# bittremieux/ANN-SoLo

Measured on AMD Instinct MI355X. Metric: query spectra/sec + recall@k vs brute-force, open-mod search on MassIVE-KB, higher is better.
Workload: dtype f32; 1 GPU; configs[2]: MassIVE-KB-scale synthetic library (2100000 spectra, one charge-2 partition), ivfpq m=32 nlist=4096 nprobe=128 k=1024, open +-500 Da, shifted dot, fragment tol 0.02 Da; library_size=2100000, batch_per_gpu=32768, reference_default_batch_size=16384, global_batch=32768, index=ivfpq, nlist=4096, nprobe=128, k=1024, parallelism=single

## Files before the change

ann_solo_amd/csrc/coarse_sparse.hip:

```cpp
#include "common.hpp"
#include "ivf_kernels.hpp"

namespace asl {

constexpr int CS_TL = 32;
constexpr int CS_NW = 16;
constexpr int CS_CAP = 64;

__global__ __launch_bounds__(256) void list_nonzeros_kernel(const float *__restrict__ xq, int nq, int d,
                                                            int64_t ldq, uint2 *__restrict__ ent,
                                                            int32_t *__restrict__ cnt,
                                                            int *__restrict__ n_over) {
  const int q = blockIdx.x * 4 + (threadIdx.x >> 6), lane = threadIdx.x & 63;
  if (q >= nq) return;
  const float *row = xq + (size_t)q * ldq;
  uint2 *out = ent + (size_t)q * CS_CAP;
  int base = 0;
  for (int j0 = 0; j0 < d; j0 += 64) {
    const int j = j0 + lane;
    const float x = j < d ? row[j] : 0.0f;
    const unsigned long long m = __ballot(x != 0.0f);
    if (x != 0.0f) {
      const int t = base + __popcll(m & ((1ull << lane) - 1ull));
      if (t < CS_CAP) out[t] = make_uint2((uint32_t)j * (CS_TL * 4), __float_as_uint(x));
    }
    base += __popcll(m);
  }
  for (int t = base + lane; t < CS_CAP; t += 64) out[t] = make_uint2(0u, 0u);
  if (lane == 0) {
    cnt[q] = base <= CS_CAP ? base : -1 - base;
    if (base > CS_CAP) atomicAdd(n_over, 1);
  }
}

typedef float cs_f2 __attribute__((ext_vector_type(2)));
typedef __attribute__((address_space(3))) cs_f2 cs_lds_f2;

#define CS_NOP2 "s_nop 1\n\t"
#define CS_ADDR_(PRE, K, ED, I)                                                          \
  asm(PRE "v_add_u32_dpp %0, %1, %2 row_newbcast:" #K " row_mask:0xf bank_mask:0xf"     \
      : "=v"(ad[I])                                                                      \
      : "v"(ED), "v"(lane_off));
#define CS_ADDR(K, ED, I) CS_ADDR_("", K, ED, I)
#define CS_FMA(K, EV, I) CS_FMA_("", K, EV, I)
#define CS_FMA_(PRE, K, EV, I)                                                           \
  asm(PRE "v_fmac_f32_dpp %0, %1, %2 row_newbcast:" #K " row_mask:0xf bank_mask:0xf"    \
      : "+v"(acc0)                                                                   \
      : "v"(EV), "v"(cv[I].x));                                                      \
  asm("v_fmac_f32_dpp %0, %1, %2 row_newbcast:" #K " row_mask:0xf bank_mask:0xf"    \
      : "+v"(acc1)                                                                   \
      : "v"(EV), "v"(cv[I].y));
#define CS_BLOCK8(K0, K1, K2, K3, K4, K5, K6, K7, ED, EV)                                       \
  {                                                                                             \
    uint32_t ad[8];                                                                             \
    cs_f2 cv[8];                                                                                \
    CS_ADDR_(CS_NOP2, K0, ED, 0) CS_ADDR(K1, ED, 1) CS_ADDR(K2, ED, 2) CS_ADDR(K3, ED, 3)                 \
    CS_ADDR(K4, ED, 4) CS_ADDR(K5, ED, 5) CS_ADDR(K6, ED, 6) CS_ADDR(K7, ED, 7)                 \
    _Pragma("unroll") for (int i_ = 0; i_ < 8; ++i_) cv[i_] = *(const cs_lds_f2 *)(uintptr_t)ad[i_]; \
    CS_FMA_(CS_NOP2, K0, EV, 0) CS_FMA(K1, EV, 1) CS_FMA(K2, EV, 2) CS_FMA(K3, EV, 3)                     \
    CS_FMA(K4, EV, 4) CS_FMA(K5, EV, 5) CS_FMA(K6, EV, 6) CS_FMA(K7, EV, 7)                     \
  }
#define CS_BLOCK8A(ED, EV) CS_BLOCK8(0, 1, 2, 3, 4, 5, 6, 7, ED, EV)
#define CS_BLOCK8B(ED, EV) CS_BLOCK8(8, 9, 10, 11, 12, 13, 14, 15, ED, EV)

__global__ __launch_bounds__(64 * CS_NW) void coarse_sparse_kernel(
    const float *__restrict__ xq, int nq, int d, int64_t ldq, const uint2 *__restrict__ ent,
    const int32_t *__restrict__ cnt, const float *__restrict__ Ct, int nlist,
    float *__restrict__ scores, int ld, const int *__restrict__ n_over, int over_max) {
  if (*n_over > over_max) return;
  extern __shared__ __attribute__((aligned(16))) char cs_smem[];
  float *tile = reinterpret_cast<float *>(cs_smem);
  const int tid = threadIdx.x, lane = tid & 63, wave = tid >> 6;
  const int l0 = blockIdx.x * CS_TL;
  if (l0 + CS_TL <= nlist && (nlist & 3) == 0) {
    for (int i = tid; i < d * (CS_TL / 4); i += 64 * CS_NW) {
      const int dim = i >> 3, l4 = (i & 7) * 4;
      reinterpret_cast<float4 *>(tile)[i] =
          *reinterpret_cast<const float4 *>(Ct + (size_t)dim * nlist + l0 + l4);
    }
  } else {
    for (int i = tid; i < d * CS_TL; i += 64 * CS_NW) {
      const int dim = i >> 5, l = i & 31;
      tile[i] = l0 + l < nlist ? Ct[(size_t)dim * nlist + l0 + l] : 0.0f;
    }
  }
  __syncthreads();
  const int row = lane >> 4, j = lane & 15;
  const char *tile_lane = reinterpret_cast<const char *>(tile) + j * 8;
  const uint32_t lane_off =
      (uint32_t)(uintptr_t)(__attribute__((address_space(3))) char *)cs_smem + (uint32_t)(j * 8);
  const int groups = (nq + 3) >> 2;
  const int gper = (groups + gridDim.y - 1) / gridDim.y;
  const int g_lo = blockIdx.y * gper, g_hi = min(groups, g_lo + gper);
  uint32_t n_ed[4] = {0u, 0u, 0u, 0u}, n_ev[4] = {0u, 0u, 0u, 0u};
  int n_c = 0;
  auto fetch = [&](int g) {
    const int q = g * 4 + row;
    if (g < g_hi && q < nq) {
      n_c = cnt[q];
      const uint2 *e = ent + (size_t)q * CS_CAP + j;
#pragma unroll
      for (int u = 0; u < 4; ++u) {
        const uint2 x = e[16 * u];
        n_ed[u] = x.x;
        n_ev[u] = x.y;
      }
    } else {
      n_c = 0;
#pragma unroll
      for (int u = 0; u < 4; ++u) n_ed[u] = n_ev[u] = 0u;
    }
  };
  fetch(g_lo + wave);
  for (int g = g_lo + wave; g < g_hi; g += CS_NW) {
    const int q = g * 4 + row;
    const bool live = q < nq;
    const int c = n_c;
    const uint32_t ed[4] = {n_ed[0], n_ed[1], n_ed[2], n_ed[3]};
    const uint32_t ev[4] = {n_ev[0], n_ev[1], n_ev[2], n_ev[3]};
    fetch(g + CS_NW);
    float acc0 = 0.0f, acc1 = 0.0f;
    int cm = c < 0 ? 0 : c;
#pragma unroll
    for (int o = 32; o > 0; o >>= 1) cm = max(cm, __shfl_xor(cm, o, 64));
    cm = __builtin_amdgcn_readfirstlane(cm);
    if (cm > 0) { CS_BLOCK8A(ed[0], ev[0]) }
    if (cm > 8) { CS_BLOCK8B(ed[0], ev[0]) }
    if (cm > 16) { CS_BLOCK8A(ed[1], ev[1]) }
    if (cm > 24) { CS_BLOCK8B(ed[1], ev[1]) }
    if (cm > 32) { CS_BLOCK8A(ed[2], ev[2]) }
    if (cm > 40) { CS_BLOCK8B(ed[2], ev[2]) }
    if (cm > 48) { CS_BLOCK8A(ed[3], ev[3]) }
    if (cm > 56) { CS_BLOCK8B(ed[3], ev[3]) }
    if (__ballot(c < 0)) {
      if (c < 0) {
        acc0 = acc1 = 0.0f;
        const float *xr = xq + (size_t)q * ldq;
        for (int k = 0; k < d; ++k) {
          const float vv = xr[k];
          if (vv != 0.0f) {
            const float2 cc = *reinterpret_cast<const float2 *>(tile_lane + (size_t)k * (CS_TL * 4));
            acc0 = __builtin_fmaf(vv, cc.x, acc0);
            acc1 = __builtin_fmaf(vv, cc.y, acc1);
          }
        }
      }
    }
    if (live) {
      const int l = l0 + 2 * j;
      float *o = scores + (size_t)q * ld + l;
      if (l + 1 < nlist && (ld & 1) == 0) {
        *reinterpret_cast<float2 *>(o) = make_float2(acc0, acc1);
      } else {
        if (l < nlist) o[0] = acc0;
        if (l + 1 < nlist) o[1] = acc1;
      }
    }
  }
}

int list_nonzeros(const float *xq, int nq, int d, int64_t ldq, uint2 *ent, int32_t *cnt, int *n_over) {
  if (nq <= 0) return ASL_OK;
  hipLaunchKernelGGL(list_nonzeros_kernel, dim3((unsigned)cdiv(nq, 4)), dim3(256), 0, stream(), xq,
                     nq, d, ldq > 0 ? ldq : (int64_t)d, ent, cnt, n_over);
  ASL_CHECK_LAUNCH();
  return ASL_OK;
}

bool coarse_sparse_supported(int d, int nlist) {
  return d >= 1 && (size_t)d * CS_TL * 4 <= 150 * 1024 && nlist >= 1;
}

__global__ void transpose_f32_kernel(const float *__restrict__ in, int rows, int cols,
                                     float *__restrict__ out) {
  __shared__ float t[32][33];
  const int bx = blockIdx.x * 32, by = blockIdx.y * 32;
  const int x = threadIdx.x & 31, y0 = threadIdx.x >> 5;
  for (int y = y0; y < 32; y += 8)
    if (by + y < rows && bx + x < cols) t[y][x] = in[(size_t)(by + y) * cols + bx + x];
  __syncthreads();
  for (int y = y0; y < 32; y += 8)
    if (bx + y < cols && by + x < rows) out[(size_t)(bx + y) * rows + by + x] = t[x][y];
}

int transpose_f32(const float *in, int rows, int cols, float *out) {
  if (rows <= 0 || cols <= 0) return ASL_OK;
  hipLaunchKernelGGL(transpose_f32_kernel, dim3((unsigned)cdiv(cols, 32), (unsigned)cdiv(rows, 32)),
                     dim3(256), 0, stream(), in, rows, cols, out);
  ASL_CHECK_LAUNCH();
  return ASL_OK;
}

int coarse_sparse(const float *xq, int nq, int d, const float *Ct, int nlist, uint2 *ent,
                  int32_t *cnt, int *n_over, int over_max, float *scores, int ld, int64_t ldq) {
  if (ldq <= 0) ldq = d;
  if (nq <= 0) return ASL_OK;
  HIP_TRY(hipMemsetAsync(n_over, 0, sizeof(int), stream()));
  hipLaunchKernelGGL(list_nonzeros_kernel, dim3((unsigned)cdiv(nq, 4)), dim3(256), 0, stream(), xq,
                     nq, d, ldq, ent, cnt, n_over);
  ASL_CHECK_LAUNCH();
  const int tiles = (int)cdiv(nlist, CS_TL);
  int parts = std::max(1, std::min((512 + tiles - 1) / tiles, (nq + 4 * CS_NW - 1) / (4 * CS_NW)));
  const size_t lds = (size_t)d * CS_TL * 4;
  HIP_TRY(hipFuncSetAttribute((const void *)coarse_sparse_kernel,
                              hipFuncAttributeMaxDynamicSharedMemorySize, (int)lds));
  hipLaunchKernelGGL(coarse_sparse_kernel, dim3(tiles, parts), dim3(64 * CS_NW), lds, stream(), xq, nq, d,
                     ldq, ent, cnt, Ct, nlist, scores, ld, n_over, over_max);
  ASL_CHECK_LAUNCH();
  return ASL_OK;
}

int coarse_sparse_cap() { return CS_CAP; }

}
```

ann_solo_amd/csrc/encode.hip:

```cpp
#include "common.hpp"

namespace asl {

__device__ __forceinline__ uint32_t rotl32(uint32_t x, int r) {
  return (x << r) | (x >> (32 - r));
}

__device__ __forceinline__ uint32_t murmur3_round(uint32_t h1, uint32_t k1) {
  k1 *= 0xcc9e2d51u;
  k1 = rotl32(k1, 15);
  k1 *= 0x1b873593u;
  h1 ^= k1;
  h1 = rotl32(h1, 13);
  return h1 * 5 + 0xe6546b64u;
}

__device__ __forceinline__ uint32_t murmur3_decimal_small(int v, uint32_t seed) {
  const bool neg = v < 0;
  uint32_t u = neg ? (uint32_t)(-(long long)v) : (uint32_t)v;
  int nd = 1;
  nd += u >= 10u;
  nd += u >= 100u;
  nd += u >= 1000u;
  nd += u >= 10000u;
  nd += u >= 100000u;
  nd += u >= 1000000u;
  nd += u >= 10000000u;
  nd += u >= 100000000u;
  const int len = nd + (neg ? 1 : 0);
  uint32_t w0 = neg ? (uint32_t)'-' : 0u, w1 = 0u, w2 = 0u;
#pragma unroll
  for (int j = 0; j < 9; ++j) {
    if (j < nd) {
      const uint32_t qd = u / 10u;
      const uint32_t ch = (uint32_t)'0' + (u - qd * 10u);
      u = qd;
      const int pos = len - 1 - j;
      const uint32_t sh = ch << ((pos & 3) * 8);
      w0 |= (pos >> 2) == 0 ? sh : 0u;
      w1 |= (pos >> 2) == 1 ? sh : 0u;
      w2 |= (pos >> 2) == 2 ? sh : 0u;
    }
  }
  uint32_t h1 = seed;
  if (len >= 4) h1 = murmur3_round(h1, w0);
  if (len >= 8) h1 = murmur3_round(h1, w1);
  const uint32_t tail = len >= 8 ? w2 : (len >= 4 ? w1 : w0);
  if (len & 3) {
    uint32_t k1 = tail & (0xFFFFFFFFu >> (32 - 8 * (len & 3)));
    k1 *= 0xcc9e2d51u;
    k1 = rotl32(k1, 15);
    k1 *= 0x1b873593u;
    h1 ^= k1;
  }
  h1 ^= (uint32_t)len;
  h1 ^= h1 >> 16;
  h1 *= 0x85ebca6bu;
  h1 ^= h1 >> 13;
  h1 *= 0xc2b2ae35u;
  h1 ^= h1 >> 16;
  return h1;
}

__device__ uint32_t murmur3_decimal(long long v, uint32_t seed) {
  if (v > -1000000000ll && v < 1000000000ll) return murmur3_decimal_small((int)v, seed);
  unsigned char buf[24];
  int len = 0;
  unsigned long long u = v < 0 ? (unsigned long long)(-(v + 1)) + 1ull : (unsigned long long)v;
  unsigned char tmp[24];
  int nd = 0;
  do {
    tmp[nd++] = (unsigned char)('0' + (u % 10));
    u /= 10;
  } while (u);
  if (v < 0) buf[len++] = '-';
  for (int i = nd - 1; i >= 0; --i) buf[len++] = tmp[i];
  const uint32_t c1 = 0xcc9e2d51u, c2 = 0x1b873593u;
  uint32_t h1 = seed;
  int nblocks = len >> 2;
  for (int i = 0; i < nblocks; ++i) {
    uint32_t k1 = (uint32_t)buf[4 * i] | ((uint32_t)buf[4 * i + 1] << 8) |
                  ((uint32_t)buf[4 * i + 2] << 16) | ((uint32_t)buf[4 * i + 3] << 24);
    k1 *= c1;
    k1 = rotl32(k1, 15);
    k1 *= c2;
    h1 ^= k1;
    h1 = rotl32(h1, 13);
    h1 = h1 * 5 + 0xe6546b64u;
  }
  uint32_t k1 = 0;
  int t = nblocks * 4;
  int rem = len & 3;
  if (rem == 3) k1 ^= (uint32_t)buf[t + 2] << 16;
  if (rem >= 2) k1 ^= (uint32_t)buf[t + 1] << 8;
  if (rem >= 1) {
    k1 ^= buf[t];
    k1 *= c1;
    k1 = rotl32(k1, 15);
    k1 *= c2;
    h1 ^= k1;
  }
  h1 ^= (uint32_t)len;
  h1 ^= h1 >> 16;
  h1 *= 0x85ebca6bu;
  h1 ^= h1 >> 13;
  h1 *= 0xc2b2ae35u;
  h1 ^= h1 >> 16;
  return h1;
}

__device__ long long np_floor_div_bin(double a, double b) {
  const double q0 = a / b;
  if (b > 0.0 && fabs(q0) < 2147483648.0) {
    double q = floor(q0);
    if (fma(-q, b, a) < 0.0) q -= 1.0;
    return (long long)q;
  }
  double mod = fmod(a, b);
  double div = (a - mod) / b;
  if (mod != 0.0 && ((b < 0) != (mod < 0))) div -= 1.0;
  double fd;
  if (div != 0.0) {
    fd = floor(div);
    if (div - fd > 0.5) fd += 1.0;
  } else {
    fd = copysign(0.0, a / b);
  }
  return (long long)floor(fd);
}

constexpr int ENC_WAVES = 4;
constexpr int QE_CAP = 64;
constexpr int QE_DIM_SHIFT = 7;

template <bool ENTRIES>
__global__ __launch_bounds__(64 * ENC_WAVES) void encode_kernel(
    const float *__restrict__ mz, const float *__restrict__ inten,
    const int32_t *__restrict__ offsets, int32_t n, double min_bound, double bin_size,
    int32_t hash_len, uint32_t seed, int norm, float *__restrict__ out, uint2 *__restrict__ ent,
    int32_t *__restrict__ ent_cnt, int *__restrict__ n_over) {
  extern __shared__ __attribute__((aligned(16))) char smem[];
  const int wave = threadIdx.x >> 6, lane = threadIdx.x & 63;
  const int spec = blockIdx.x * ENC_WAVES + wave;
  float *vec = reinterpret_cast<float *>(smem) + (size_t)wave * hash_len;
  if (spec >= n) return;

  for (int i = lane; i < hash_len; i += 64) vec[i] = 0.0f;
  const int p0 = offsets[spec], p1 = offsets[spec + 1];
  for (int base = p0; base < p1; base += 64) {
    const int p = base + lane;
    const int cnt = min(64, p1 - base);
    const bool live = lane < cnt;
    int idx = -1 - lane;
    float val = 0.0f;
    if (live) {
      long long b = np_floor_div_bin((double)mz[p] - min_bound, bin_size);
      idx = (int)(murmur3_decimal(b, seed) % (uint32_t)hash_len);
      val = inten[p];
    }
    int rank = 0;
    for (int j = 0; j < cnt; ++j) {
      const int o = __builtin_amdgcn_readlane(idx, j);
      rank += (o == idx && j < lane) ? 1 : 0;
    }
    for (int r = 0; __ballot(live && rank >= r) != 0ull; ++r) {
      if (live && rank == r) vec[idx] += val;
      __builtin_amdgcn_wave_barrier();
    }
  }
  float nrm = 1.0f;
  if (norm) {
    float acc = 0.0f;
    for (int i0 = 0; i0 < hash_len; i0 += 64) {
      const int i = i0 + lane;
      const float v = i < hash_len ? vec[i] : 0.0f;
      unsigned long long m = __ballot(v != 0.0f);
      while (m) {
        const int l = __builtin_ctzll(m);
        m &= m - 1ull;
        const float x = __builtin_bit_cast(
            float, __builtin_amdgcn_readlane(__builtin_bit_cast(int, v), l));
        acc = __builtin_fmaf(x, x, acc);
      }
    }
    nrm = __builtin_sqrtf(acc);
  }
  if (!ENTRIES) {
    float *row = out + (size_t)spec * hash_len;
    for (int i = lane; i < hash_len; i += 64) row[i] = norm ? vec[i] / nrm : vec[i];
    return;
  }
  uint2 *row = ent + (size_t)spec * QE_CAP;
  int have = 0;
  for (int i0 = 0; i0 < hash_len; i0 += 64) {
    const int i = i0 + lane;
    float x = i < hash_len ? vec[i] : 0.0f;
    if (norm) x = x / nrm;
    if (!(i < hash_len)) x = 0.0f;
    const unsigned long long m = __ballot(x != 0.0f);
    if (x != 0.0f) {
      const int t = have + __popcll(m & ((1ull << lane) - 1ull));
      if (t < QE_CAP) row[t] = make_uint2((uint32_t)i << QE_DIM_SHIFT, __float_as_uint(x));
    }
    have += __popcll(m);
  }
  for (int t = have + lane; t < QE_CAP; t += 64) row[t] = make_uint2(0u, 0u);
  if (lane == 0) {
    ent_cnt[spec] = have <= QE_CAP ? have : -1 - have;
    if (have > QE_CAP && n_over) atomicAdd(n_over, 1);
  }
}

template <bool ENTRIES>
static int encode_launch(const float *mz, const float *inten, const int32_t *offsets, int32_t n,
                         double min_bound, double bin_size, int32_t hash_len, uint32_t seed, int norm,
                         float *out, uint2 *ent, int32_t *ent_cnt, int *n_over) {
  size_t lds = (size_t)ENC_WAVES * hash_len * sizeof(float);
  if (lds > 160 * 1024) return fail(ASL_ERR_CAPACITY, "encode: hash_len %d too large for LDS", hash_len);
  dim3 grid((unsigned)cdiv(n, ENC_WAVES));
  if (lds > 64 * 1024)
    HIP_TRY(hipFuncSetAttribute((const void *)encode_kernel<ENTRIES>,
                                hipFuncAttributeMaxDynamicSharedMemorySize, (int)lds));
  hipLaunchKernelGGL(encode_kernel<ENTRIES>, grid, dim3(64 * ENC_WAVES), lds, stream(), mz, inten,
                     offsets, n, min_bound, bin_size, hash_len, seed, norm, out, ent, ent_cnt, n_over);
  ASL_CHECK_LAUNCH();
  return ASL_OK;
}

int encode_device(const float *mz, const float *inten, const int32_t *offsets, int32_t n,
                  double min_bound, double bin_size, int32_t hash_len, uint32_t seed,
                  int norm, float *out) {
  if (n == 0) return ASL_OK;
  ProfScope ps("encode");
  return encode_launch<false>(mz, inten, offsets, n, min_bound, bin_size, hash_len, seed, norm, out,
                              nullptr, nullptr, nullptr);
}

int encode_entries_device(const float *mz, const float *inten, const int32_t *offsets, int32_t n,
                          double min_bound, double bin_size, int32_t hash_len, uint32_t seed, int norm,
                          uint2 *ent, int32_t *cnt, int *n_over) {
  if (n == 0) return ASL_OK;
  ProfScope ps("encode");
  return encode_launch<true>(mz, inten, offsets, n, min_bound, bin_size, hash_len, seed, norm, nullptr,
                             ent, cnt, n_over);
}

}

using namespace asl;

static uint32_t host_rotl32(uint32_t x, int r) { return (x << r) | (x >> (32 - r)); }
static uint32_t host_murmur3(const unsigned char *key, int len, uint32_t seed) {
  const uint32_t c1 = 0xcc9e2d51u, c2 = 0x1b873593u;
  uint32_t h1 = seed;
  int nblocks = len / 4;
  for (int i = 0; i < nblocks; i++) {
    uint32_t k1;
    memcpy(&k1, key + 4 * i, 4);
    k1 *= c1;
    k1 = host_rotl32(k1, 15);
    k1 *= c2;
    h1 ^= k1;
    h1 = host_rotl32(h1, 13);
    h1 = h1 * 5 + 0xe6546b64u;
  }
  const unsigned char *tail = key + nblocks * 4;
  uint32_t k1 = 0;
  switch (len & 3) {
    case 3: k1 ^= (uint32_t)tail[2] << 16; [[fallthrough]];
    case 2: k1 ^= (uint32_t)tail[1] << 8; [[fallthrough]];
    case 1:
      k1 ^= tail[0];
      k1 *= c1;
      k1 = host_rotl32(k1, 15);
      k1 *= c2;
      h1 ^= k1;
  }
  h1 ^= (uint32_t)len;
  h1 ^= h1 >> 16;
  h1 *= 0x85ebca6bu;
  h1 ^= h1 >> 13;
  h1 *= 0xc2b2ae35u;
  h1 ^= h1 >> 16;
  return h1;
}

extern "C" {

int32_t asl_hash_idx(int64_t bin_idx, int32_t hash_len, uint32_t seed) {
  if (hash_len <= 0) return -1;
  char buf[32];
  int len = snprintf(buf, sizeof buf, "%lld", (long long)bin_idx);
  return (int32_t)(host_murmur3((const unsigned char *)buf, len, seed) % (uint32_t)hash_len);
}

int asl_get_dim(double min_mz, double max_mz, double bin_size, int64_t *n_bins,
                double *start_dim, double *end_dim) {
  if (!(bin_size > 0)) return fail(ASL_ERR_INVALID, "get_dim: bin_size must be > 0");
  auto pymod = [](double a, double b) {
    double m = fmod(a, b);
    if (m != 0.0 && ((b < 0) != (m < 0))) m += b;
    return m;
  };
  double s = min_mz - pymod(min_mz, bin_size);
  double e = max_mz + bin_size - pymod(max_mz, bin_size);
  if (start_dim) *start_dim = s;
  if (end_dim) *end_dim = e;
  if (n_bins) *n_bins = (int64_t)nearbyint((e - s) / bin_size);
  return ASL_OK;
}

int asl_encode_batch(const float *mz, const float *intensity, const int32_t *offsets,
                     int32_t n, double min_bound, double bin_size, int32_t hash_len,
                     uint32_t seed, int norm, float *out) {
  clear_error();
  if (n < 0 || hash_len <= 0 || !(bin_size > 0))
    return fail(ASL_ERR_INVALID, "encode_batch: bad n/hash_len/bin_size");
  if (n == 0) return ASL_OK;
  if (!offsets || !out) return fail(ASL_ERR_INVALID, "encode_batch: null offsets/out");
  ASL_TRY(ensure_device());
  int32_t last = 0;
  if (is_device_ptr(offsets)) {
    HIP_TRY(hipMemcpyAsync(&last, offsets + n, sizeof(int32_t), hipMemcpyDeviceToHost, stream()));
    ASL_TRY(sync_stream());
  } else {
    last = offsets[n];
  }
  if (last > 0 && (!mz || !intensity)) return fail(ASL_ERR_INVALID, "encode_batch: null peaks");
  In<float> dmz, din;
  In<int32_t> doff;
  Out<float> dout;
  ASL_TRY(dmz.init(mz, (size_t)last));
  ASL_TRY(din.init(intensity, (size_t)last));
  ASL_TRY(doff.init(offsets, (size_t)n + 1));
  ASL_TRY(dout.init(out, (size_t)n * hash_len));
  ASL_TRY(encode_device(dmz.d, din.d, doff.d, n, min_bound, bin_size, hash_len, seed, norm,
                        dout.d));
  ASL_TRY(dout.finish());
  if (dout.to_host() || dmz.own.p || din.own.p || doff.own.p) ASL_TRY(sync_stream());
  return ASL_OK;
}

int asl_encode_entries_batch(const float *mz, const float *intensity, const int32_t *offsets,
                             int32_t n, int32_t n_peaks, double min_bound, double bin_size,
                             int32_t hash_len, uint32_t seed, int norm, uint32_t *entries,
                             int32_t *counts, int32_t *n_over) {
  clear_error();
  if (n < 0 || hash_len <= 0 || !(bin_size > 0))
    return fail(ASL_ERR_INVALID, "encode_entries_batch: bad n/hash_len/bin_size");
  if (n == 0) return ASL_OK;
  if (!offsets || !entries || !counts) return fail(ASL_ERR_INVALID, "encode_entries_batch: null offsets/entries/counts");
  ASL_TRY(ensure_device());
  if (!is_device_ptr(entries) || !is_device_ptr(counts) || (n_over && !is_device_ptr(n_over)))
    return fail(ASL_ERR_INVALID, "encode_entries_batch: entries / counts / n_over must be device memory");
  int32_t last = n_peaks;
  if (last < 0) {
    if (is_device_ptr(offsets)) {
      HIP_TRY(hipMemcpyAsync(&last, offsets + n, sizeof(int32_t), hipMemcpyDeviceToHost, stream()));
      ASL_TRY(sync_stream());
    } else {
      last = offsets[n];
    }
  }
  if (last > 0 && (!mz || !intensity)) return fail(ASL_ERR_INVALID, "encode_entries_batch: null peaks");
  In<float> dmz, din;
  In<int32_t> doff;
  ASL_TRY(dmz.init(mz, (size_t)last));
  ASL_TRY(din.init(intensity, (size_t)last));
  ASL_TRY(doff.init(offsets, (size_t)n + 1));
  ASL_TRY(encode_entries_device(dmz.d, din.d, doff.d, n, min_bound, bin_size, hash_len, seed, norm,
                                reinterpret_cast<uint2 *>(entries), counts, n_over));
  if (dmz.own.p || din.own.p || doff.own.p) ASL_TRY(sync_stream());
  return ASL_OK;
}

}
```

ann_solo_amd/csrc/index.hpp:

```cpp
#pragma once
#include "common.hpp"
#include "flat_postings.hpp"
#include "ivf_kernels.hpp"

namespace asl {

constexpr size_t SCORE_CHUNK_BYTES = (size_t)1 << 30;
constexpr int FLAT_KEYS_SLACK = 768;

struct ShardScratch {
  DevBuf<float> x_all, cD, cD_all, Dp, Dr, Dtmp, Dfin, x3, cD3;
  DevBuf<int32_t> cI, cI_all, cI3, mine, everyone;
  DevBuf<int64_t> Ip, Ir, Im;
  DevBuf<uint2> e_loc, e_all, e3;
  DevBuf<int32_t> c_loc, c_all, c3, over;
  DevBuf<int64_t> Kp, Hs, Hr, Ko, Bs, Br, Xs, Xr, Mn, rowlist, K3;
  DevBuf<int32_t> need, flag, Fl, rmap;
  DevBuf<unsigned int> cursor;
};

enum IndexRows { ROWS_ORDERED = 0, ROWS_SET, ROWS_SET_RAW, ROWS_KEYS };

struct IndexSearch {
  int nq = 0;
  const float *xq = nullptr;
  int k = 0, nprobe = 0;
  float *D = nullptr;
  int64_t *I64 = nullptr;
  int32_t *I32 = nullptr;
  const float *pre_D = nullptr;
  const int32_t *pre_I = nullptr;
  const uint2 *pre_ent = nullptr;
  const int32_t *pre_cnt = nullptr;
  const int *gate = nullptr;
  int rows = ROWS_ORDERED;
  const IndexPostFilter *post = nullptr;
  uint64_t serial = 0, gen = 0;
  const IndexWindow *win = nullptr;
  const uint8_t *sel_keep = nullptr;
  int64_t sel_n = 0;
  bool rows_filtered = false;
};

}

struct asl_index {
  int d = 0, nlist = 0, kind = 0, pq_m = 0, pq_bits = 8, ksub = 0, dsub = 0;
  int niter = 25;
  bool trained = false;
  bool by_residual = true;
  int64_t ntotal = 0;
  int64_t n_store = 0;
  int shard_rank = 0, shard_world = 1;
  asl::DevBuf<float> centroids, codebooks;
  asl::DevBuf<float> codebooks_t;
  bool cbt_ready = false;
  asl::DevBuf<float> centroids_t;
  bool cent_t_ready = false;
  asl::DevBuf<float> kmeans_ct;
  asl::DevBuf<uint2> scan_ent;
  asl::DevBuf<int32_t> scan_cnt;
  asl::DevBuf<int> scan_over;
  asl::DevBuf<uint2> cs_ent;
  asl::DevBuf<int32_t> cs_cnt;
  asl::DevBuf<int> cs_over;
  asl::DevBuf<float> vecs;
  asl::DevBuf<int32_t> vlist;
  asl::DevBuf<int32_t> vids;
  bool has_vids = false;
  asl::DevBuf<uint8_t> codes_add;
  asl::DevBuf<uint8_t> codes;
  asl::DevBuf<int32_t> ids, list_offsets;
  std::vector<int32_t> h_list_offsets;
  asl::DevBuf<uint8_t> codes_tiled;
  asl::DevBuf<int32_t> ids_tiled, tile_offsets;
  asl::DevBuf<int2> idpay;
  int64_t n_tile_slots = 0;
  uint64_t pay_serial = 0;
  uint64_t pay_gen = 0;
  int64_t pay_n = 0;
  bool idpay_ready = false;
  bool has_tiles = false;
  asl::DevBuf<uint8_t> wcodes_tiled;
  asl::DevBuf<int32_t> wids_tiled;
  asl::DevBuf<float> wkey_tiled;
  bool win_ready = false;
  uint64_t win_serial = 0;
  uint64_t win_gen = 0;
  int window_scan = 0;
  asl::DevBuf<int2> win_ranges;
  asl::DevBuf<float> wf_key;
  asl::DevBuf<uint8_t> codes_mm;
  uint32_t mm_plane = 0;
  bool mm_ready = false;
  bool scan_mmajor = true;
  asl::DevBuf<unsigned long long> sel_words, wsel_words;
  bool sel_ready = false, wsel_ready = false;
  uint64_t sel_serial = 0, sel_gen = 0, wsel_serial = 0, wsel_gen = 0;
  asl::DevBuf<uint8_t> selector;
  bool has_selector = false;
  uint64_t selector_gen = 0;
  int64_t n_blocks = 0;
  asl::DevBuf<int32_t> blk_offsets;
  asl::DevBuf<uint32_t> blk_base;
  asl::DevBuf<uint32_t> inv_tab;
  asl::DevBuf<char> inv_data;
  bool has_inv = false;
  int flat_storage = ASL_FLAT_F32;
  int inv_layout = 0;
  int nnz_max = 0;
  int tab_stride = 0;
  asl::DevBuf<uint8_t> inv_tab8;
  asl::DevBuf<uint16_t> inv_cnt16;
  int scan_variant = 0;
  int unordered = 0;
  bool lists_dirty = true;
  int agreed_k = -1, agreed_np = -1, agreed_world = -1, agreed_val = -1;
  int refine_k = 0;
  bool refine_rows = false;
  bool refine_bad = false;
  int64_t r_n = 0;
  asl::DevBuf<uint16_t> r_dim;
  asl::DevBuf<float> r_val;
  asl::DevBuf<uint8_t> r_cnt;
  asl::DevBuf<int32_t> ws_short;
  asl::DevBuf<float> ws_scores, coarse_D, ws_x;
  asl::DevBuf<int32_t> coarse_I, ws_assign;
  asl::DevBuf<float> zero_D;
  asl::DevBuf<uint32_t> bitmap;
  asl::DevBuf<uint64_t> ws_upper;
  asl::ShardScratch shard;
};

namespace asl {

int index_shape_check(const char *who, int d, int nlist, int kind, int pq_m, int pq_bits);
constexpr int PQ_TILED_MAX_D = 1020;
inline bool ivf_kind(int kind) { return kind == ASL_INDEX_IVFFLAT || kind == ASL_INDEX_IVFPQ; }
inline bool window_mode(const asl_index *ix) { return ix->window_scan || ix->kind == ASL_INDEX_WINFLAT; }
inline bool tiled_index(const asl_index *ix) {
  return ix->kind == ASL_INDEX_IVFPQ && ix->pq_m == 32 && ix->ksub == 256 && ix->d <= PQ_TILED_MAX_D;
}
inline FlatPostings postings_view(const asl_index *ix) {
  FlatPostings P;
  P.layout = ix->has_inv ? ix->inv_layout : 0, P.d = ix->d, P.nlist = ix->nlist, P.n_blocks = ix->n_blocks;
  P.list_offsets = ix->list_offsets.p, P.blk_offsets = ix->blk_offsets.p, P.blk_base = ix->blk_base.p;
  if (P.layout == 2) P.tab8 = ix->inv_tab8.p, P.cnt16 = ix->inv_cnt16.p;
  else P.tab32 = ix->inv_tab.p;
  P.tab_stride = ix->tab_stride, P.seg_bytes = ix->inv_data.p, P.ids = ix->ids.p;
  return P;
}
int assign_ip(asl_index *ix, const float *x, int64_t ld, int64_t n, const float *cent, int k, int d,
              int32_t *assign_dev);
int build_lists(asl_index *ix);
int build_postings(asl_index *ix, const int32_t *order_dev, int64_t n, const std::vector<int32_t> &blk_off,
                   const std::vector<int32_t> &pos_blk, const std::vector<uint16_t> &pos_loc);
int winflat_layout(asl_index *ix, bool keyed, const float *key, uint64_t serial, uint64_t gen);
const char *window_unsupported(const asl_index *ix);
int window_install(asl_index *ix, int64_t n, const float *key, uint64_t serial, uint64_t gen = 0);
int post_filter_pairs(asl_index *ix, const IndexPostFilter &p, uint64_t serial, uint64_t gen,
                      const int32_t *slot_ids, int64_t nslots);
int selector_words(asl_index *ix, const IndexSearch &rq, bool window, const unsigned long long **words);
int index_search_device(asl_index *ix, IndexSearch &rq);
int index_nprobe(const asl_index *ix, int nprobe);
int index_prepare(asl_index *ix);
int coarse_search(asl_index *ix, const float *xq, int nq, int nprobe, float *out_D, int32_t *out_I, uint2 *ent_out,
                  int32_t *cnt_out, bool *have_ent);
int index_window_prepare(asl_index *ix, uint64_t serial, uint64_t gen, const float *key, int64_t n, int nq,
                         int nprobe);
int index_refine_k(const asl_index *ix);
int coarse_scores_all(asl_index *ix, const float *xq, int m, float *scores, uint2 *ent = nullptr, int32_t *cnt = nullptr);
int index_codebooks_transposed(asl_index *ix);
int index_codes_mmajor(asl_index *ix);
int index_zero_coarse(asl_index *ix, size_t n, const float **zeros);

}
```

ann_solo_amd/csrc/index_search.hip:

```cpp
#include <algorithm>

#include "index.hpp"

namespace asl {

static int coarse_transposed(asl_index *ix) {
  if (ix->cent_t_ready) return ASL_OK;
  ASL_TRY(ix->centroids_t.reserve((size_t)ix->nlist * ix->d));
  ASL_TRY(transpose_f32(ix->centroids.p, ix->nlist, ix->d, ix->centroids_t.p));
  ix->cent_t_ready = true;
  return ASL_OK;
}

int coarse_scores_all(asl_index *ix, const float *xq, int m, float *scores, uint2 *ent, int32_t *cnt) {
  const int nlist = ix->nlist, d = ix->d;
  const bool sparse = ix->scan_variant == 0 && coarse_sparse_supported(d, nlist);
  const int over_max = m / 64;
  if (sparse) {
    ASL_TRY(coarse_transposed(ix));
    ASL_TRY(ix->cs_ent.reserve((size_t)m * coarse_sparse_cap()));
    ASL_TRY(ix->cs_cnt.reserve((size_t)m));
    ASL_TRY(ix->cs_over.reserve(1));
    ASL_TRY(coarse_sparse(xq, m, d, ix->centroids_t.p, nlist, ent ? ent : ix->cs_ent.p, cnt ? cnt : ix->cs_cnt.p,
                          ix->cs_over.p, over_max, scores, nlist));
  }
  return gemm_nt_f32(xq, ix->centroids.p, scores, m, nlist, d, d, d, nlist, sparse ? ix->cs_over.p : nullptr, over_max);
}

int coarse_search(asl_index *ix, const float *xq, int nq, int nprobe, float *out_D, int32_t *out_I, uint2 *ent_out,
                  int32_t *cnt_out, bool *have_ent) {
  const int nlist = ix->nlist, d = ix->d;
  if (have_ent) *have_ent = false;
  if (!out_D) {
    ASL_TRY(ix->coarse_D.reserve((size_t)nq * nprobe));
    ASL_TRY(ix->coarse_I.reserve((size_t)nq * nprobe));
    out_D = ix->coarse_D.p;
    out_I = ix->coarse_I.p;
  }
  int rows = (int)std::min<int64_t>(nq, std::max<int64_t>(1, (int64_t)(SCORE_CHUNK_BYTES / ((size_t)nlist * 4))));
  ASL_TRY(ix->ws_scores.reserve((size_t)rows * nlist));
  const bool sparse = ix->scan_variant == 0 && coarse_sparse_supported(d, nlist);
  for (int r0 = 0; r0 < nq; r0 += rows) {
    const int m = std::min(rows, nq - r0);
    {
      ProfScope ps("coarse_gemm");
      ASL_TRY(coarse_scores_all(ix, xq + (size_t)r0 * d, m, ix->ws_scores.p, ent_out ? ent_out + (size_t)r0 * 64 : nullptr,
                                cnt_out ? cnt_out + (size_t)r0 : nullptr));
    }
    {
      ProfScope ps("coarse_select");
      ASL_TRY(row_topk(ix->ws_scores.p, nlist, m, nlist, nprobe, nullptr, 0, nullptr, nullptr, 0,
                       out_D + (size_t)r0 * nprobe, nullptr, out_I + (size_t)r0 * nprobe, nprobe));
    }
  }
  if (have_ent) *have_ent = sparse && coarse_sparse_cap() == 64 && ((ent_out && cnt_out) || nq <= rows);
  return ASL_OK;
}

static bool postings_ok(const asl_index *ix, int k, int nprobe) {
  return ix->has_inv && ix->scan_variant == 0 && flat_inv_supported(ix->d, k, nprobe);
}
static bool tiled_shape_ok(const asl_index *ix, int k, int nprobe) {
  return ix->scan_variant == 0 && tiled_index(ix) && pq_scan_tiled_supported(ix->pq_m, ix->ksub, k, nprobe);
}
static bool keys_fit(int k) { return k + FLAT_KEYS_SLACK <= TK_MAX_K; }

static int clamp_nprobe(const asl_index *ix, int *nprobe, const char *who) {
  *nprobe = std::max(1, std::min(*nprobe, ix->nlist));
  if (*nprobe > TK_MAX_K) return fail(ASL_ERR_CAPACITY, "%s: nprobe=%d > %d", who, *nprobe, TK_MAX_K);
  return ASL_OK;
}

static int count_scanned(const asl_index *ix, const int32_t *cI, int nq, int nprobe) {
  if (!prof_counts()) return ASL_OK;
  if (unsigned long long *acc = prof_scanned_dev())
    ASL_TRY(scanned_count(cI, (int64_t)nq * nprobe, ix->list_offsets.p, acc));
  return ASL_OK;
}

struct SearchPlan {
  int unordered = 0;
  int nprobe = 0;
  bool refine = false;
  int k_scan = 0;
  bool use_inv = false, tiled = false;
};

static int validate_winflat(asl_index *ix, const IndexSearch &rq, const SearchPlan &pl) {
  if (rq.gate || rq.pre_I || rq.pre_D)
    return fail(ASL_ERR_STATE, "a window-exact index has no probe lists: no preassigned or gated search");
  if (rq.pre_ent && !rq.xq) return fail(ASL_ERR_STATE, "a window-exact index takes no entry-list-only queries");
  if (pl.unordered == 2) return fail(ASL_ERR_STATE, "packed-key rows are not served by a window-exact index");
  if (rq.sel_keep && !rq.win)
    return fail(ASL_ERR_STATE, "a window-exact index takes a selection through its key column (NaN: unselected), "
                               "not a selector");
  if (rq.win && !rq.win->q_pmz) return fail(ASL_ERR_INVALID, "window scan: null precursor m/z");
  if (rq.nq <= 0) return ASL_OK;
  if (!rq.xq) return fail(ASL_ERR_INVALID, "search: null queries");
  if (rq.k <= 0) return fail(ASL_ERR_CAPACITY, "search: k=%d outside 1..%d", rq.k, TK_MAX_K - FLAT_KEYS_SLACK);
  if (!keys_fit(rq.k))
    return fail(ASL_ERR_STATE, "a window-exact index holds k <= %d (k=%d)", TK_MAX_K - FLAT_KEYS_SLACK, rq.k);
  if (!flat_inv_supported(ix->d, rq.k, 1))
    return fail(ASL_ERR_STATE, "a window-exact index is searched by the postings scan, which holds d <= 4096 (d=%d)", ix->d);
  ASL_TRY(build_lists(ix));
  if (ix->n_store > 0 && !ix->has_inv && ix->d <= 65535 && ix->nnz_max == 0)
    return fail(ASL_ERR_STATE, "a window-exact index of all-zero vectors has no postings to scan");
  if (ix->n_store > 0 && !ix->has_inv)
    return fail(ASL_ERR_STATE, "a window-exact index needs sparse vectors: its postings are built when the most "
                               "non-zeros of a vector (%d), times 8, stay below d=%d", ix->nnz_max, ix->d);
  if (rq.win && !ix->win_ready)
    return fail(ASL_ERR_STATE, "window scan: no window key (asl_index_set_window_key), or vectors were added "
                               "since it was set");
  return ASL_OK;
}

static int validate(asl_index *ix, const IndexSearch &rq, SearchPlan &pl) {
  const int k = rq.k;
  pl.unordered = rq.rows == ROWS_KEYS ? 2 : rq.rows == ROWS_SET_RAW ? 1 : ix->unordered;
  if (ix->kind == ASL_INDEX_WINFLAT) return validate_winflat(ix, rq, pl);
  pl.refine = ix->kind == ASL_INDEX_IVFPQ && ix->refine_k > k && ix->refine_rows && pl.unordered == 0;
  if (rq.win) {
    if (const char *why = window_unsupported(ix)) return fail(ASL_ERR_STATE, "%s", why);
    if (ix->scan_variant != 0)
      return fail(ASL_ERR_STATE, "the window scan needs the layout-specific scan (scan_variant 0), not the generic kernels");
    if (!keys_fit(k)) return fail(ASL_ERR_STATE, "the window scan holds k <= %d (k=%d)", TK_MAX_K - FLAT_KEYS_SLACK, k);
    if (rq.gate || pl.unordered == 2 || pl.refine)
      return fail(ASL_ERR_STATE, "the window scan takes no gate, packed keys or exact re-rank");
    if (!rq.win->q_pmz) return fail(ASL_ERR_INVALID, "window scan: null precursor m/z");
  }
  if (rq.sel_keep) {
    if (ix->kind == ASL_INDEX_FLAT) return fail(ASL_ERR_STATE, "a selector needs an IVF index (not a Flat index)");
    if (ix->shard_world > 1 || ix->has_vids) return fail(ASL_ERR_STATE, "a selector does not run on a sharded index");
    if (ix->scan_variant != 0)
      return fail(ASL_ERR_STATE, "a selector needs the layout-specific scan (scan_variant 0), not the generic kernels");
    if (!keys_fit(k)) return fail(ASL_ERR_STATE, "a selected search holds k <= %d (k=%d)", TK_MAX_K - FLAT_KEYS_SLACK, k);
    if (rq.gate || pl.unordered == 2 || (rq.pre_ent && !rq.xq))
      return fail(ASL_ERR_STATE, "a selected search takes no gate, packed keys or entry-list-only queries");
    if (pl.refine) return fail(ASL_ERR_STATE, "a selected search does not run with the exact re-rank");
    if (rq.sel_n != ix->ntotal)
      return fail(ASL_ERR_INVALID, "selector: %lld flags for %lld vectors", (long long)rq.sel_n, (long long)ix->ntotal);
  }
  if (rq.nq <= 0) return ASL_OK;
  if (rq.pre_ent && (!rq.pre_cnt || !rq.pre_I || (!rq.xq && !rq.pre_D) || ix->kind == ASL_INDEX_FLAT))
    return fail(ASL_ERR_STATE, "entry-list search: needs the counts, the caller's probe lists (with their scores when "
                               "no dense rows are given) and an IVF index");
  if (!rq.xq && !rq.pre_ent) return fail(ASL_ERR_INVALID, "search: null queries");
  if (rq.gate && (!rq.pre_I || ix->kind == ASL_INDEX_FLAT))
    return fail(ASL_ERR_STATE, "gated search: needs the caller's probe lists and an IVF index");
  if (!ix->trained) return fail(ASL_ERR_STATE, "search: index is not trained");
  if (k <= 0 || k > TK_MAX_K_PASSES) return fail(ASL_ERR_CAPACITY, "search: k=%d outside 1..%d", k, TK_MAX_K_PASSES);
  const bool ents_only = rq.pre_ent && !rq.xq;
  pl.nprobe = rq.nprobe;
  pl.k_scan = k;
  if (k > TK_MAX_K && (rq.gate || ents_only || pl.unordered == 2))
    return fail(ASL_ERR_STATE, "search: k=%d > %d is served from dense queries only (no packed keys, "
                               "entry-list-only queries or gates)", k, TK_MAX_K);
  if (ix->kind == ASL_INDEX_FLAT) {
    if (pl.unordered == 2) return fail(ASL_ERR_STATE, "packed-key rows need an IVF index");
    return ASL_OK;
  }
  ASL_TRY(clamp_nprobe(ix, &pl.nprobe, "search"));
  ASL_TRY(build_lists(ix));
  if (k > TK_MAX_K) return ASL_OK;
  if (ix->kind == ASL_INDEX_IVFFLAT) {
    pl.use_inv = postings_ok(ix, k, pl.nprobe);
    if (pl.unordered == 2 && !(pl.use_inv && rq.I64 && keys_fit(k)))
      return fail(ASL_ERR_STATE, "packed-key rows need the postings scan of IVF-Flat (sparse vectors, k <= 1280) and an int64 output");
    if (rq.gate && !pl.use_inv) return fail(ASL_ERR_STATE, "gated search: needs the postings scan of IVF-Flat");
    if (ents_only && !pl.use_inv) return fail(ASL_ERR_STATE, "entry-list search: needs the postings scan of IVF-Flat");
    if (rq.sel_keep && !pl.use_inv)
      return fail(ASL_ERR_STATE, "a selector needs the postings scan of IVF-Flat (sparse vectors, nprobe <= 1024), "
                                 "not dense rows");
    return ASL_OK;
  }
  if (rq.gate && pl.refine) return fail(ASL_ERR_STATE, "gated search: not with the exact re-rank");
  if (ents_only && pl.refine) return fail(ASL_ERR_STATE, "entry-list search: not with the exact re-rank (it reads the dense queries)");
  if (pl.refine) {
    if (ix->refine_bad)
      return fail(ASL_ERR_CAPACITY, "search: refine is unavailable, a stored vector has more than %d non-zeros",
                  refine_stride());
    if (ix->r_n != ix->ntotal)
      return fail(ASL_ERR_STATE, "search: refine rows cover %lld of %lld vectors (enable refine before add)",
                  (long long)ix->r_n, (long long)ix->ntotal);
    pl.k_scan = std::min(ix->refine_k, (int)TK_MAX_K);
  }
  pl.tiled = ix->has_tiles && tiled_shape_ok(ix, pl.k_scan, pl.nprobe);
  if (pl.unordered == 2 && !(pl.tiled && rq.I64))
    return fail(ASL_ERR_STATE, "packed-key rows need the tiled IVF-PQ scan (m = 32, 8 bits) and an int64 output");
  if (rq.gate && !pl.tiled) return fail(ASL_ERR_STATE, "gated search: needs the tiled IVF-PQ scan");
  if (ents_only && !pl.tiled) return fail(ASL_ERR_STATE, "entry-list search: needs the tiled IVF-PQ scan (m = 32, 8 bits)");
  if (rq.sel_keep && !pl.tiled)
    return fail(ASL_ERR_STATE, "a selector needs the tiled IVF-PQ scan (m = 32, 8 bits, nprobe <= 1024)");
  if (rq.win && !pl.tiled) return fail(ASL_ERR_STATE, "the window scan needs the tiled IVF-PQ scan (m = 32, 8 bits)");
  if (rq.win && !ix->win_ready)
    return fail(ASL_ERR_STATE, "window scan: no window key (asl_index_set_window_key), or the lists changed "
                               "since it was set");
  return ASL_OK;
}

static int query_entries(asl_index *ix, const IndexSearch &rq, bool own_ent, const uint2 **q_ent,
                         const int32_t **q_cnt) {
  *q_ent = rq.pre_ent;
  *q_cnt = rq.pre_cnt;
  if (!rq.pre_ent && own_ent) {
    *q_ent = ix->cs_ent.p;
    *q_cnt = ix->cs_cnt.p;
  } else if (!rq.pre_ent) {
    ASL_TRY(ix->scan_ent.reserve((size_t)rq.nq * 64));
    ASL_TRY(ix->scan_cnt.reserve((size_t)rq.nq));
    ASL_TRY(ix->scan_over.reserve(1));
    ASL_TRY(list_nonzeros(rq.xq, rq.nq, ix->d, ix->d, ix->scan_ent.p, ix->scan_cnt.p, ix->scan_over.p));
    *q_ent = ix->scan_ent.p;
    *q_cnt = ix->scan_cnt.p;
  }
  return ASL_OK;
}

static int take_post_filter(asl_index *ix, IndexSearch &rq, int mode, const int32_t *slot_ids, int64_t nslots,
                            ScanPostFilter &pf) {
  pf = ScanPostFilter();
  if (!rq.post) return ASL_OK;
  const IndexPostFilter &p = *rq.post;
  if (!(mode == 1 && rq.I32 && !rq.I64 && !rq.D && !rq.gate && keys_fit(rq.k)) || !p.payload || !p.q_pmz || !p.count ||
      p.n != ix->ntotal || ix->has_vids) return ASL_OK;
  ASL_TRY(post_filter_pairs(ix, p, rq.serial, rq.gen, slot_ids, nslots));
  pf = {.idpay = ix->idpay.p, .q_pmz = p.q_pmz, .count = p.count, .tol = p.tol, .mode = p.mode, .charge = p.charge};
  rq.rows_filtered = true;
  return ASL_OK;
}

static int pass_bounds(asl_index *ix, const IndexSearch &rq, uint64_t **upper) {
  *upper = nullptr;
  if (rq.k <= TK_MAX_K) return ASL_OK;
  ASL_TRY(ix->ws_upper.reserve((size_t)rq.nq));
  *upper = ix->ws_upper.p;
  return ASL_OK;
}

static int search_gemm_topk(asl_index *ix, const IndexSearch &rq, const int32_t *cI, int nprobe) {
  const int nq = rq.nq, k = rq.k, d = ix->d;
  const int64_t n = ix->n_store;
  const bool ivf = cI != nullptr;
  uint64_t *upper;
  ASL_TRY(pass_bounds(ix, rq, &upper));
  int words = 0;
  if (ivf) {
    words = (ix->nlist + 31) / 32;
    ASL_TRY(ix->bitmap.reserve((size_t)nq * words));
    ASL_TRY(probe_bitmap(cI, nq, nprobe, ix->bitmap.p, words));
    if (n > 0) ASL_TRY(count_scanned(ix, cI, nq, nprobe));
  }
  const int64_t ncol = std::max<int64_t>(n, 1);
  int rows = (int)std::min<int64_t>(nq, std::max<int64_t>(1, (int64_t)(SCORE_CHUNK_BYTES / ((size_t)ncol * 4))));
  ASL_TRY(ix->ws_scores.reserve((size_t)rows * ncol));
  auto out_at = [&](auto *base, int64_t r0, int c0) { return base ? base + (size_t)r0 * k + c0 : nullptr; };
  for (int r0 = 0; r0 < nq; r0 += rows) {
    const int m = std::min(rows, nq - r0);
    ProfScope ps("scan");
    if (n > 0)
      ASL_TRY(gemm_nt_f32(rq.xq + (size_t)r0 * d, ix->vecs.p, ix->ws_scores.p, m, (int)n, d, d, d, (int)n));
    for (int c0 = 0; c0 < k; c0 += TK_MAX_K) {
      const int kp = std::min<int>(TK_MAX_K, k - c0);
      ASL_TRY(row_topk(ix->ws_scores.p, n, m, (int)n, kp, ix->has_vids ? ix->vids.p : nullptr, 0,
                       ivf ? ix->vlist.p : nullptr, ivf ? ix->bitmap.p + (size_t)r0 * words : nullptr, words,
                       out_at(rq.D, r0, c0), out_at(rq.I64, r0, c0), out_at(rq.I32, r0, c0), k,
                       c0 ? upper + r0 : nullptr, upper ? upper + r0 : nullptr));
    }
  }
  return upper ? sync_stream() : ASL_OK;
}

static int search_ivfflat(asl_index *ix, IndexSearch &rq, const SearchPlan &pl) {
  const int nq = rq.nq, nprobe = pl.nprobe;
  bool own_ent = false;
  if (!rq.pre_I) ASL_TRY(coarse_search(ix, rq.xq, nq, nprobe, nullptr, nullptr, nullptr, nullptr, &own_ent));
  const int32_t *cI = rq.pre_I ? rq.pre_I : ix->coarse_I.p;
  if (!pl.use_inv) return search_gemm_topk(ix, rq, cI, nprobe);
  const uint2 *q_ent;
  const int32_t *q_cnt;
  ASL_TRY(query_entries(ix, rq, own_ent, &q_ent, &q_cnt));
  const int mode_ = pl.unordered ? pl.unordered : (rq.rows != ROWS_ORDERED ? 1 : 0);
  ScanPostFilter pf;
  ASL_TRY(take_post_filter(ix, rq, mode_, ix->ids.p, ix->n_store, pf));
  const unsigned long long *sel = nullptr;
  if (rq.sel_keep) ASL_TRY(selector_words(ix, rq, false, &sel));
  {
    ProfScope ps("scan");
    FlatScan fs;
    fs.xq = rq.xq, fs.ent = q_ent, fs.ent_cnt = q_cnt, fs.nq = nq, fs.k = rq.k;
    fs.coarse_I = cI, fs.nprobe = nprobe, fs.gate = rq.gate, fs.post = pf, fs.sel = sel;
    fs.D = rq.D, fs.I64 = rq.I64, fs.I32 = rq.I32, fs.set_mode = mode_;
    ASL_TRY(flat_inv_scan(postings_view(ix), fs));
  }
  return rq.gate ? ASL_OK : count_scanned(ix, cI, nq, nprobe);
}

static int search_winflat(asl_index *ix, IndexSearch &rq, const SearchPlan &pl) {
  const int nq = rq.nq;
  const uint2 *q_ent;
  const int32_t *q_cnt;
  ASL_TRY(query_entries(ix, rq, false, &q_ent, &q_cnt));
  const int mode_ = (pl.unordered || rq.rows != ROWS_ORDERED) ? 1 : 0;
  ASL_TRY(ix->win_ranges.reserve((size_t)nq));
  {
    ProfScope ps("window_ranges");
    const IndexWindow *w = rq.win;
    ASL_TRY(winflat_runs(w ? w->q_pmz : nullptr, nq, ix->wf_key.p, ix->n_store, w ? w->charge : 0, w ? w->tol : 0.0,
                         w ? w->mode : ASL_TOL_DA, ix->win_ranges.p,
                         prof_counts() ? prof_scanned_dev() : nullptr));
  }
  FlatScan fs;
  fs.xq = rq.xq, fs.ent = q_ent, fs.ent_cnt = q_cnt, fs.nq = nq, fs.k = rq.k;
  fs.D = rq.D, fs.I64 = rq.I64, fs.I32 = rq.I32, fs.set_mode = mode_;
  fs.ranges.range = ix->win_ranges.p;
  fs.ranges.row_len = (rq.win && mode_ == 1) ? rq.win->row_len : nullptr;
  rq.rows_filtered = fs.ranges.row_len != nullptr;
  ProfScope ps("scan");
  return flat_inv_scan(postings_view(ix), fs);
}

int index_codebooks_transposed(asl_index *ix) {
  if (ix->cbt_ready) return ASL_OK;
  const size_t ncb = (size_t)ix->pq_m * ix->ksub * ix->dsub;
  std::vector<float> h((size_t)ncb), ht((size_t)ncb);
  ASL_TRY(ix->codebooks.download(h.data(), ncb));
  ASL_TRY(sync_stream());
  for (int m = 0; m < ix->pq_m; m++)
    for (int c = 0; c < ix->ksub; c++)
      for (int t = 0; t < ix->dsub; t++)
        ht[((size_t)m * ix->dsub + t) * ix->ksub + c] = h[((size_t)m * ix->ksub + c) * ix->dsub + t];
  ASL_TRY(ix->codebooks_t.upload(ht.data(), ncb));
  ASL_TRY(sync_stream());
  ix->cbt_ready = true;
  return ASL_OK;
}

int index_zero_coarse(asl_index *ix, size_t n, const float **zeros) {
  if (n > ix->zero_D.cap) {
    ASL_TRY(ix->zero_D.reserve(n));
    HIP_TRY(hipMemsetAsync(ix->zero_D.p, 0, n * sizeof(float), stream()));
  }
  *zeros = ix->zero_D.p;
  return ASL_OK;
}

int index_codes_mmajor(asl_index *ix) {
  if (ix->mm_ready) return ASL_OK;
  const int64_t ntiles = ix->n_tile_slots / 64;
  const uint64_t plane = ((((uint64_t)ntiles * 64 + 127) / 128) | 1u) * 128;
  if (plane * (uint64_t)ix->pq_m >= (1ull << 32)) return ASL_OK;
  ASL_TRY(ix->codes_mm.reserve((size_t)plane * (size_t)ix->pq_m));
  ASL_TRY(mmajor_codes(ix->codes_tiled.p, ntiles, (uint32_t)plane, ix->codes_mm.p));
  ASL_TRY(sync_stream());
  ix->mm_plane = (uint32_t)plane;
  ix->mm_ready = true;
  return ASL_OK;
}

static int scan_pq_tiled(asl_index *ix, IndexSearch &rq, const SearchPlan &pl, const float *cD, const int32_t *cI,
                         bool own_ent) {
  const int nq = rq.nq, nprobe = pl.nprobe;
  ASL_TRY(index_codebooks_transposed(ix));
  const uint2 *q_ent;
  const int32_t *q_cnt;
  ASL_TRY(query_entries(ix, rq, own_ent, &q_ent, &q_cnt));
  const int mode_ = pl.unordered ? pl.unordered : (rq.rows != ROWS_ORDERED ? 1 : 0);
  ScanPostFilter pf;
  ScanRanges rg;
  if (rq.win) {
    const IndexWindow &wq = *rq.win;
    ASL_TRY(ix->win_ranges.reserve((size_t)nq * nprobe));
    ProfScope ps("window_ranges");
    ASL_TRY(window_ranges(wq.q_pmz, nq, cI, nprobe, ix->list_offsets.p, ix->tile_offsets.p, ix->wkey_tiled.p,
                          wq.charge, wq.tol, wq.mode, ix->win_ranges.p,
                          prof_counts() ? prof_scanned_dev() : nullptr));
    rg.range = ix->win_ranges.p;
    rg.row_len = mode_ == 1 ? wq.row_len : nullptr;
    rq.rows_filtered = rg.row_len != nullptr;
  } else {
    ASL_TRY(take_post_filter(ix, rq, mode_, ix->ids_tiled.p, ix->n_tile_slots, pf));
  }
  const unsigned long long *sel = nullptr;
  if (rq.sel_keep) ASL_TRY(selector_words(ix, rq, rq.win != nullptr, &sel));
  const bool mm = ix->scan_mmajor && !rq.win && !rq.sel_keep && !rq.gate && ix->shard_world == 1 && !ix->has_vids;
  if (mm) ASL_TRY(index_codes_mmajor(ix));
  const bool use_mm = mm && ix->mm_ready;
  ProfScope ps("scan");
  return pq_scan_v3(rq.xq, nq, ix->d, ix->codebooks_t.p, ix->dsub, cD, cI,
                    nprobe, ix->list_offsets.p, ix->tile_offsets.p,
                    rq.win ? ix->wcodes_tiled.p : ix->codes_tiled.p, rq.win ? ix->wids_tiled.p : ix->ids_tiled.p,
                    rq.k, rq.D, rq.I64, rq.I32, mode_, q_ent, q_cnt, rq.gate, &pf, &rg, sel,
                    use_mm ? ix->codes_mm.p : nullptr, use_mm ? ix->mm_plane : 0u);
}

static int search_ivfpq(asl_index *ix, IndexSearch &rq, const SearchPlan &pl) {
  const int nq = rq.nq, nprobe = pl.nprobe;
  bool own_ent = false;
  if (!rq.pre_D) ASL_TRY(coarse_search(ix, rq.xq, nq, nprobe, nullptr, nullptr, nullptr, nullptr, &own_ent));
  const float *cD = rq.pre_D ? rq.pre_D : ix->coarse_D.p;
  const int32_t *cI = rq.pre_D ? rq.pre_I : ix->coarse_I.p;
  if (!ix->by_residual) ASL_TRY(index_zero_coarse(ix, (size_t)nq * nprobe, &cD));
  uint64_t *upper = nullptr;
  if (pl.tiled) {
    ASL_TRY(scan_pq_tiled(ix, rq, pl, cD, cI, own_ent));
  } else {
    const int k = rq.k;
    ASL_TRY(pass_bounds(ix, rq, &upper));
    auto out_at = [&](auto *base, int c0) { return base ? base + c0 : nullptr; };
    ProfScope ps("scan");
    for (int c0 = 0; c0 < k; c0 += TK_MAX_K) {
      const int kp = std::min<int>(TK_MAX_K, k - c0);
      ASL_TRY(pq_scan(rq.xq, nq, ix->d, ix->codebooks.p, ix->pq_m, ix->ksub, ix->dsub, cD, cI, nprobe,
                      ix->list_offsets.p, ix->ids.p, ix->codes.p, kp, out_at(rq.D, c0), out_at(rq.I64, c0),
                      out_at(rq.I32, c0), k, c0 ? upper : nullptr, upper));
    }
  }
  if (!rq.gate && !rq.win) ASL_TRY(count_scanned(ix, cI, nq, nprobe));
  return upper ? sync_stream() : ASL_OK;
}

static int search_ivfpq_refined(asl_index *ix, IndexSearch &rq, const SearchPlan &pl) {
  IndexSearch scan = rq;
  scan.k = pl.k_scan;
  ASL_TRY(ix->ws_short.reserve((size_t)rq.nq * scan.k));
  scan.D = nullptr;
  scan.I64 = nullptr;
  scan.I32 = ix->ws_short.p;
  scan.rows = ROWS_SET;
  scan.post = nullptr;
  ASL_TRY(search_ivfpq(ix, scan, pl));
  ProfScope ps("refine");
  return refine_topk(rq.xq, rq.nq, ix->d, ix->ws_short.p, nullptr, scan.k, ix->r_dim.p, ix->r_val.p, ix->r_cnt.p,
                     ix->r_n, rq.k, rq.D, rq.I64, rq.I32);
}

int index_search_device(asl_index *ix, IndexSearch &rq) {
  rq.rows_filtered = false;
  SearchPlan pl;
  ASL_TRY(validate(ix, rq, pl));
  if (rq.nq <= 0) return ASL_OK;
  if (ix->kind == ASL_INDEX_FLAT) return search_gemm_topk(ix, rq, nullptr, 0);
  if (ix->kind == ASL_INDEX_WINFLAT) return search_winflat(ix, rq, pl);
  if (ix->kind == ASL_INDEX_IVFFLAT) return search_ivfflat(ix, rq, pl);
  return pl.refine ? search_ivfpq_refined(ix, rq, pl) : search_ivfpq(ix, rq, pl);
}

int index_window_prepare(asl_index *ix, uint64_t serial, uint64_t gen, const float *key, int64_t n, int nq,
                         int nprobe) {
  if (!ix->trained) return fail(ASL_ERR_STATE, "search: index is not trained");
  if (ix->kind != ASL_INDEX_WINFLAT) ASL_TRY(build_lists(ix));
  if (ix->lists_dirty || !ix->win_ready || ix->win_serial != serial || ix->win_gen != gen) {
    ASL_TRY(pipeline_drain());
    ASL_TRY(window_install(ix, n, key, serial, gen));
  }
  return ix->win_ranges.reserve((size_t)std::max(nq, 1) * std::max(1, std::min(nprobe, ix->nlist)));
}

int index_nprobe(const asl_index *ix, int nprobe) {
  return !ivf_kind(ix->kind) ? 0 : std::max(1, std::min(nprobe, ix->nlist));
}
int index_prepare(asl_index *ix) {
  if (!ix->trained) return fail(ASL_ERR_STATE, "search: index is not trained");
  if (!ivf_kind(ix->kind)) return ASL_OK;
  if (coarse_sparse_supported(ix->d, ix->nlist)) ASL_TRY(coarse_transposed(ix));
  return build_lists(ix);
}
int index_refine_k(const asl_index *ix) {
  return (ix->refine_rows && !ix->refine_bad && ix->r_n == ix->ntotal) ? ix->refine_k : 0;
}

template <class F>
static int with_staged_rows(float *D, int64_t *I, size_t n, bool staged_in, F call) {
  Out<float> dD;
  Out<int64_t> dI;
  ASL_TRY(dD.init(D, n));
  ASL_TRY(dI.init(I, n));
  ASL_TRY(call(dD.d, dI.d));
  ASL_TRY(dD.finish());
  ASL_TRY(dI.finish());
  if (dD.to_host() || dI.to_host() || staged_in) ASL_TRY(sync_stream());
  return ASL_OK;
}

}

using namespace asl;

extern "C" {

int asl_index_supports_keys(asl_index_t *ix, int32_t k, int32_t nprobe) {
  if (!ix) return 0;
  nprobe = std::max(1, std::min(nprobe, ix->nlist));
  if (ix->kind == ASL_INDEX_IVFFLAT) {
    if (ix->lists_dirty && ix->trained && (ensure_device() != ASL_OK || build_lists(ix) != ASL_OK)) return 0;
    return postings_ok(ix, k, nprobe) && keys_fit(k);
  }
  if (ix->kind != ASL_INDEX_IVFPQ) return 0;
  return tiled_shape_ok(ix, k, nprobe) && keys_fit(k);
}

int asl_index_coarse(asl_index_t *ix, int32_t nq, const float *xq, int32_t nprobe,
                     float *coarse_D, int32_t *coarse_I) {
  clear_error();
  if (!ix || !ivf_kind(ix->kind) || !ix->trained)
    return fail(ASL_ERR_STATE, "coarse: trained IVF index required");
  if (nq <= 0) return ASL_OK;
  ASL_TRY(clamp_nprobe(ix, &nprobe, "coarse"));
  In<float> dq;
  ASL_TRY(dq.init(xq, (size_t)nq * ix->d));
  ASL_TRY(coarse_search(ix, dq.d, nq, nprobe, nullptr, nullptr, nullptr, nullptr, nullptr));
  if (coarse_D)
    HIP_TRY(hipMemcpyAsync(coarse_D, ix->coarse_D.p, (size_t)nq * nprobe * 4, hipMemcpyDefault, stream()));
  if (coarse_I)
    HIP_TRY(hipMemcpyAsync(coarse_I, ix->coarse_I.p, (size_t)nq * nprobe * 4, hipMemcpyDefault, stream()));
  return sync_stream();
}

int asl_index_postings_work(asl_index_t *ix, int32_t nq, const float *xq, int32_t nprobe,
                            int64_t *bytes, int64_t *lines) {
  clear_error();
  if (!ix || ix->kind != ASL_INDEX_IVFFLAT || !ix->trained)
    return fail(ASL_ERR_STATE, "postings_work: trained IVF-Flat index required");
  if (bytes) *bytes = 0;
  if (lines) *lines = 0;
  if (nq <= 0) return ASL_OK;
  ASL_TRY(ensure_device());
  ASL_TRY(clamp_nprobe(ix, &nprobe, "postings_work"));
  ASL_TRY(build_lists(ix));
  if (!ix->has_inv) return fail(ASL_ERR_STATE, "postings_work: the index holds no postings (dense vectors)");
  In<float> dq;
  ASL_TRY(dq.init(xq, (size_t)nq * ix->d));
  ASL_TRY(coarse_search(ix, dq.d, nq, nprobe, nullptr, nullptr, nullptr, nullptr, nullptr));
  DevBuf<unsigned long long> acc;
  ASL_TRY(acc.reserve(2));
  HIP_TRY(hipMemsetAsync(acc.p, 0, 16, stream()));
  ASL_TRY(flat_postings_work(postings_view(ix), dq.d, nq, ix->coarse_I.p, nprobe, acc.p));
  unsigned long long h[2] = {0, 0};
  ASL_TRY(acc.download(h, 2));
  ASL_TRY(sync_stream());
  if (bytes) *bytes = (int64_t)h[0];
  if (lines) *lines = (int64_t)h[1];
  return ASL_OK;
}

int asl_index_pq_lut(asl_index_t *ix, int32_t nq, const float *xq, float *lut) {
  clear_error();
  if (!ix || ix->kind != ASL_INDEX_IVFPQ || !ix->trained)
    return fail(ASL_ERR_STATE, "pq_lut: trained IVF-PQ index required");
  if (nq <= 0) return ASL_OK;
  In<float> dq;
  Out<float> dl;
  ASL_TRY(dq.init(xq, (size_t)nq * ix->d));
  ASL_TRY(dl.init(lut, (size_t)nq * ix->pq_m * ix->ksub));
  ASL_TRY(pq_lut(dq.d, nq, ix->d, ix->codebooks.p, ix->pq_m, ix->ksub, ix->dsub, dl.d));
  ASL_TRY(dl.finish());
  return sync_stream();
}

int asl_index_search(asl_index_t *ix, int32_t nq, const float *xq, int32_t k, int32_t nprobe,
                     float *D, int64_t *I) {
  clear_error();
  if (!ix) return fail(ASL_ERR_INVALID, "search: null index");
  if (nq <= 0) return ASL_OK;
  if (!xq || !I) return fail(ASL_ERR_INVALID, "search: null xq / I");
  ASL_TRY(ensure_device());
  In<float> dq;
  ASL_TRY(dq.init(xq, (size_t)nq * ix->d));
  return with_staged_rows(D, I, (size_t)nq * k, dq.own.p, [&](float *dD, int64_t *dI) {
    IndexSearch rq{.nq = nq, .xq = dq.d, .k = k, .nprobe = nprobe, .D = dD, .I64 = dI};
    return index_search_device(ix, rq);
  });
}

int asl_index_search_window(asl_index_t *ix, int32_t nq, const float *xq, const double *q_pmz, int32_t charge,
                            double tol, int32_t mode, int32_t k, int32_t nprobe, float *D, int64_t *I) {
  clear_error();
  ASL_TRY(ensure_device());
  if (!ix) return fail(ASL_ERR_INVALID, "search_window: null index");
  if (nq <= 0) return ASL_OK;
  if (!xq || !q_pmz || !I) return fail(ASL_ERR_INVALID, "search_window: null xq / q_pmz / I");
  if (mode != ASL_TOL_DA && mode != ASL_TOL_PPM && mode != ASL_TOL_INTERVAL)
    return fail(ASL_ERR_INVALID, "search_window: mode must be Da, ppm or interval");
  if (ix->kind != ASL_INDEX_WINFLAT)
    if (const char *why = window_unsupported(ix)) return fail(ASL_ERR_STATE, "%s", why);
  if (!ix->trained) return fail(ASL_ERR_STATE, "search: index is not trained");
  if (ix->kind != ASL_INDEX_WINFLAT || !ix->lists_dirty) ASL_TRY(build_lists(ix));
  if (!ix->win_ready || (ix->kind == ASL_INDEX_WINFLAT && ix->lists_dirty))
    return fail(ASL_ERR_STATE, "search_window: no window key (asl_index_set_window_key), or the lists changed since");
  In<float> dq;
  In<double> dp;
  ASL_TRY(dq.init(xq, (size_t)nq * ix->d));
  ASL_TRY(dp.init(q_pmz, (size_t)nq * (mode == ASL_TOL_INTERVAL ? 2 : 1)));
  return with_staged_rows(D, I, (size_t)nq * k, dq.own.p || dp.own.p, [&](float *dD, int64_t *dI) {
    IndexWindow w{.q_pmz = dp.d, .tol = tol, .mode = mode, .charge = charge};
    IndexSearch rq{.nq = nq, .xq = dq.d, .k = k, .nprobe = nprobe, .D = dD, .I64 = dI, .win = &w};
    return index_search_device(ix, rq);
  });
}

int asl_index_set_selector(asl_index_t *ix, int64_t n, const uint8_t *keep) {
  clear_error();
  ASL_TRY(ensure_device());
  if (!ix) return fail(ASL_ERR_INVALID, "set_selector: null index");
  if (n == 0 || !keep) {
    ix->has_selector = false;
    return ASL_OK;
  }
  if (n != ix->ntotal)
    return fail(ASL_ERR_INVALID, "set_selector: %lld flags for %lld vectors", (long long)n, (long long)ix->ntotal);
  if (ivf_kind(ix->kind) && ix->trained) ASL_TRY(build_lists(ix));
  ix->has_selector = false;
  ASL_TRY(ix->selector.reserve((size_t)n));
  HIP_TRY(hipMemcpyAsync(ix->selector.p, keep, (size_t)n, hipMemcpyDefault, stream()));
  ASL_TRY(sync_stream());
  ix->has_selector = true;
  ++ix->selector_gen;
  return ASL_OK;
}

int asl_index_search_selected(asl_index_t *ix, int32_t nq, const float *xq, const double *q_pmz, int32_t charge,
                              double tol, int32_t mode, int32_t k, int32_t nprobe, float *D, int64_t *I) {
  clear_error();
  ASL_TRY(ensure_device());
  if (!ix) return fail(ASL_ERR_INVALID, "search_selected: null index");
  if (nq <= 0) return ASL_OK;
  if (!xq || !I) return fail(ASL_ERR_INVALID, "search_selected: null xq / I");
  if (q_pmz && mode != ASL_TOL_DA && mode != ASL_TOL_PPM && mode != ASL_TOL_INTERVAL)
    return fail(ASL_ERR_INVALID, "search_selected: mode must be Da, ppm or interval");
  if (ix->kind == ASL_INDEX_FLAT) return fail(ASL_ERR_STATE, "a selector needs an IVF index (not a Flat index)");
  if (ix->kind == ASL_INDEX_WINFLAT)
    return fail(ASL_ERR_STATE, "search_selected: a window-exact index takes a selection through its key column "
                               "(NaN: unselected), not a selector");
  if (!ix->trained) return fail(ASL_ERR_STATE, "search: index is not trained");
  ASL_TRY(build_lists(ix));
  if (!ix->has_selector)
    return fail(ASL_ERR_STATE, "search_selected: no selector (asl_index_set_selector), or the lists changed since "
                               "it was set");
  if (q_pmz) {
    if (const char *why = window_unsupported(ix)) return fail(ASL_ERR_STATE, "%s", why);
    if (!ix->win_ready)
      return fail(ASL_ERR_STATE, "search_selected: no window key (asl_index_set_window_key), or the lists changed since");
  }
  In<float> dq;
  In<double> dp;
  ASL_TRY(dq.init(xq, (size_t)nq * ix->d));
  if (q_pmz) ASL_TRY(dp.init(q_pmz, (size_t)nq * (mode == ASL_TOL_INTERVAL ? 2 : 1)));
  return with_staged_rows(D, I, (size_t)nq * k, dq.own.p || dp.own.p, [&](float *dD, int64_t *dI) {
    IndexWindow w{.q_pmz = dp.d, .tol = tol, .mode = mode, .charge = charge};
    IndexSearch rq{.nq = nq, .xq = dq.d, .k = k, .nprobe = nprobe, .D = dD, .I64 = dI, .serial = 0,
                   .gen = ix->selector_gen, .win = q_pmz ? &w : nullptr, .sel_keep = ix->selector.p, .sel_n = ix->ntotal};
    return index_search_device(ix, rq);
  });
}

int asl_index_search_preassigned(asl_index_t *ix, int32_t nq, const float *xq, int32_t k,
                                 int32_t nprobe, const float *coarse_D,
                                 const int32_t *coarse_I, float *D, int64_t *I) {
  clear_error();
  if (ix && ix->kind == ASL_INDEX_WINFLAT)
    return fail(ASL_ERR_STATE, "search_preassigned: a window-exact index has no probe lists");
  if (!ix || ix->kind == ASL_INDEX_FLAT)
    return fail(ASL_ERR_INVALID, "search_preassigned: IVF index required");
  if (nq <= 0) return ASL_OK;
  if (!xq || !I || !coarse_D || !coarse_I) return fail(ASL_ERR_INVALID, "search_preassigned: null argument");
  if (nprobe < 1 || nprobe > ix->nlist) return fail(ASL_ERR_INVALID, "search_preassigned: nprobe outside 1..nlist");
  ASL_TRY(ensure_device());
  In<float> dq, dcD;
  In<int32_t> dcI;
  ASL_TRY(dq.init(xq, (size_t)nq * ix->d));
  ASL_TRY(dcD.init(coarse_D, (size_t)nq * nprobe));
  ASL_TRY(dcI.init(coarse_I, (size_t)nq * nprobe));
  return with_staged_rows(D, I, (size_t)nq * k, dq.own.p || dcD.own.p || dcI.own.p, [&](float *dD, int64_t *dI) {
    IndexSearch rq{.nq = nq, .xq = dq.d, .k = k, .nprobe = nprobe, .D = dD, .I64 = dI, .pre_D = dcD.d, .pre_I = dcI.d};
    return index_search_device(ix, rq);
  });
}

int asl_index_search_gated(asl_index_t *ix, int32_t cap, const float *xq, int32_t k, int32_t nprobe,
                           const float *coarse_D, const int32_t *coarse_I, float *D, int64_t *I,
                           const int32_t *count) {
  clear_error();
  if (ix && ix->kind == ASL_INDEX_WINFLAT)
    return fail(ASL_ERR_STATE, "search_gated: a window-exact index has no probe lists");
  if (!ix || ix->kind == ASL_INDEX_FLAT) return fail(ASL_ERR_INVALID, "search_gated: IVF index required");
  if (cap <= 0) return ASL_OK;
  if (!xq || !I || !coarse_D || !coarse_I || !count) return fail(ASL_ERR_INVALID, "search_gated: null argument");
  if (nprobe < 1 || nprobe > ix->nlist) return fail(ASL_ERR_INVALID, "search_gated: nprobe outside 1..nlist");
  ASL_TRY(ensure_device());
  if (!is_device_ptr(xq) || !is_device_ptr(I) || !is_device_ptr(coarse_D) || !is_device_ptr(coarse_I) ||
      !is_device_ptr(count) || (D && !is_device_ptr(D)))
    return fail(ASL_ERR_INVALID, "search_gated: device pointers only");
  IndexSearch rq{.nq = cap, .xq = xq, .k = k, .nprobe = nprobe, .D = D, .I64 = I, .pre_D = coarse_D, .pre_I = coarse_I,
                 .gate = reinterpret_cast<const int *>(count)};
  return index_search_device(ix, rq);
}

int asl_index_search_entries(asl_index_t *ix, int32_t nq, const uint32_t *entries, const int32_t *counts,
                             int32_t k, int32_t nprobe, const float *coarse_D, const int32_t *coarse_I,
                             float *D, int64_t *I, const int32_t *count) {
  clear_error();
  if (ix && ix->kind == ASL_INDEX_WINFLAT)
    return fail(ASL_ERR_STATE, "search_entries: a window-exact index has no probe lists");
  if (!ix || ix->kind == ASL_INDEX_FLAT) return fail(ASL_ERR_INVALID, "search_entries: IVF index required");
  if (nq <= 0) return ASL_OK;
  if (!entries || !counts || !I || !coarse_D || !coarse_I) return fail(ASL_ERR_INVALID, "search_entries: null argument");
  if (nprobe < 1 || nprobe > ix->nlist) return fail(ASL_ERR_INVALID, "search_entries: nprobe outside 1..nlist");
  ASL_TRY(ensure_device());
  if (!is_device_ptr(entries) || !is_device_ptr(counts) || !is_device_ptr(I) || !is_device_ptr(coarse_D) ||
      !is_device_ptr(coarse_I) || (count && !is_device_ptr(count)) || (D && !is_device_ptr(D)))
    return fail(ASL_ERR_INVALID, "search_entries: device pointers only");
  IndexSearch rq{.nq = nq, .k = k, .nprobe = nprobe, .D = D, .I64 = I, .pre_D = coarse_D, .pre_I = coarse_I,
                 .pre_ent = reinterpret_cast<const uint2 *>(entries), .pre_cnt = counts,
                 .gate = reinterpret_cast<const int *>(count)};
  return index_search_device(ix, rq);
}

int asl_index_refine(asl_index_t *ix, int32_t nq, const float *xq, int32_t kp, const int64_t *I_in,
                     int32_t k, float *D, int64_t *I) {
  clear_error();
  if (!ix || !xq || !I_in || !I) return fail(ASL_ERR_INVALID, "refine: null argument");
  if (!ix->refine_rows || ix->r_n != ix->ntotal)
    return fail(ASL_ERR_STATE, "refine: the index stores no exact rows (asl_index_set_refine before add)");
  if (ix->refine_bad) return fail(ASL_ERR_CAPACITY, "refine: a stored vector has more than %d non-zeros", refine_stride());
  if (nq <= 0) return ASL_OK;
  if (k <= 0 || k > kp || kp > TK_MAX_K) return fail(ASL_ERR_INVALID, "refine: need 0 < k <= k' <= %d", TK_MAX_K);
  ASL_TRY(ensure_device());
  In<float> dq;
  In<int64_t> dI;
  ASL_TRY(dq.init(xq, (size_t)nq * ix->d));
  ASL_TRY(dI.init(I_in, (size_t)nq * kp));
  return with_staged_rows(D, I, (size_t)nq * k, dq.own.p || dI.own.p, [&](float *oD, int64_t *oI) {
    return refine_topk(dq.d, nq, ix->d, nullptr, dI.d, kp, ix->r_dim.p, ix->r_val.p, ix->r_cnt.p, ix->r_n, k, oD, oI,
                       nullptr);
  });
}

int asl_topk_merge(int32_t S, int32_t nq, int32_t k, const float *Ds, const int64_t *Is,
                   float *D, int64_t *I) {
  clear_error();
  if (S <= 0 || nq < 0 || k <= 0 || !Ds || !Is || !D || !I) return fail(ASL_ERR_INVALID, "topk_merge: bad arguments");
  if (nq == 0) return ASL_OK;
  ASL_TRY(ensure_device());
  In<float> dDs;
  In<int64_t> dIs;
  ASL_TRY(dDs.init(Ds, (size_t)S * nq * k));
  ASL_TRY(dIs.init(Is, (size_t)S * nq * k));
  return with_staged_rows(D, I, (size_t)nq * k, dDs.own.p || dIs.own.p, [&](float *dD, int64_t *dI) {
    return topk_merge(dDs.d, dIs.d, S, nq, k, dD, dI);
  });
}

int asl_topk_merge_keys(int32_t S, int32_t nq, int32_t k, const int64_t *Ks, float *D, int64_t *I,
                        int32_t unordered) {
  clear_error();
  if (S <= 0 || nq < 0 || k <= 0 || !Ks || !I) return fail(ASL_ERR_INVALID, "topk_merge_keys: bad arguments");
  if (nq == 0) return ASL_OK;
  ASL_TRY(ensure_device());
  In<int64_t> dKs;
  ASL_TRY(dKs.init(Ks, (size_t)S * nq * k));
  return with_staged_rows(D, I, (size_t)nq * k, dKs.own.p, [&](float *dD, int64_t *dI) {
    return topk_merge_keys(dKs.d, S, nq, k, dD, dI, unordered ? 1 : 0);
  });
}

}
```

ann_solo_amd/csrc/ivf_kernels.hip:

```cpp
#include <algorithm>
#include <type_traits>

#include "common.hpp"
#include "ivf_kernels.hpp"
#include "hist_topk.hpp"
#include "topk.hpp"

namespace asl {

__global__ __launch_bounds__(TK_NT) void row_topk_kernel(
    const float *__restrict__ scores, int64_t ld, int n, int k, int cap,
    const int32_t *__restrict__ ids, int32_t id_base, const int32_t *__restrict__ vlist,
    const uint32_t *__restrict__ bitmap, int bitmap_words, float *__restrict__ D,
    int64_t *__restrict__ I64, int32_t *__restrict__ I32, int64_t out_ld,
    const u64 *__restrict__ upper_in, u64 *__restrict__ upper_out) {
  extern __shared__ __attribute__((aligned(16))) char smem[];
  u64 *buf = reinterpret_cast<u64 *>(smem);
  u64 *thr = buf + cap;
  int *ctl = reinterpret_cast<int *>(thr + 1);
  const int tid = threadIdx.x;
  const int r = blockIdx.x;
  StreamTopK<TK_NT> tk;
  tk.init(buf, ctl, thr, cap, k, tid);
  const float *row = scores + (size_t)r * ld;
  const uint32_t *bm = bitmap ? bitmap + (size_t)r * bitmap_words : nullptr;
  const u64 ub = upper_in ? upper_in[r] : ~0ull;
  for (int base = 0; base < n; base += TK_NT) {
    const int c = base + tid;
    u64 key = 0ull;
    if (c < n) {
      bool vis = true;
      if (bm) {
        const int l = vlist[c];
        vis = (bm[l >> 5] >> (l & 31)) & 1u;
      }
      if (vis) key = make_key(row[c], (uint32_t)(ids ? ids[c] : id_base + c));
      if (key >= ub) key = 0ull;
    }
    tk.push(key, tid);
  }
  tk.finish(D ? D + (size_t)r * out_ld : nullptr, I64 ? I64 + (size_t)r * out_ld : nullptr,
            I32 ? I32 + (size_t)r * out_ld : nullptr, tid);
  if (upper_out && tid == 0) upper_out[r] = ctl[0] >= k ? buf[k - 1] : 0ull;
}

constexpr int SEL_VPT = 16, SEL_CAP = 512, SEL_NB = 512;

__global__ __launch_bounds__(TK_NT) void row_select_kernel(
    const float *__restrict__ scores, int64_t ld, int n, int k, int cap, float *__restrict__ D,
    int64_t *__restrict__ I64, int32_t *__restrict__ I32, int64_t out_ld) {
  extern __shared__ __attribute__((aligned(16))) char smem[];
  u64 *buf = reinterpret_cast<u64 *>(smem);
  const int nkeys = cap > SEL_CAP ? cap : SEL_CAP;
  u64 *thr = buf + nkeys;
  int *ctl = reinterpret_cast<int *>(thr + 1);
  int *hist = ctl + 12;
  float *red = reinterpret_cast<float *>(hist + SEL_NB);
  const int tid = threadIdx.x, lane = tid & 63, wave = tid >> 6, r = blockIdx.x;
  const float *row = scores + (size_t)r * ld;
  float v[SEL_VPT];
  float lo = 3.402823466e+38f, hi = -3.402823466e+38f;
#pragma unroll
  for (int u = 0; u < SEL_VPT; ++u) {
    const int c = tid + u * TK_NT;
    v[u] = c < n ? row[c] : 0.0f;
    if (c < n) {
      lo = fminf(lo, v[u]);
      hi = fmaxf(hi, v[u]);
    }
  }
#pragma unroll
  for (int o = 32; o > 0; o >>= 1) {
    lo = fminf(lo, __shfl_xor(lo, o, 64));
    hi = fmaxf(hi, __shfl_xor(hi, o, 64));
  }
  if (lane == 0) {
    red[wave] = lo;
    red[4 + wave] = hi;
  }
  for (int i = tid; i < SEL_NB; i += TK_NT) hist[i] = 0;
  __syncthreads();
  lo = fminf(fminf(red[0], red[1]), fminf(red[2], red[3]));
  hi = fmaxf(fmaxf(red[4], red[5]), fmaxf(red[6], red[7]));
  const float scale = hi > lo ? (float)(SEL_NB - 1) / (hi - lo) : 0.0f;
  int bk[SEL_VPT];
#pragma unroll
  for (int u = 0; u < SEL_VPT; ++u) {
    const int c = tid + u * TK_NT;
    float t = (v[u] - lo) * scale;
    t = fminf(fmaxf(t, 0.0f), (float)(SEL_NB - 1));
    bk[u] = (int)t;
    if (c < n) atomicAdd(&hist[bk[u]], 1);
  }
  __syncthreads();
  {
    const int h0 = hist[SEL_NB - 1 - 2 * tid], h1 = hist[SEL_NB - 2 - 2 * tid];
    int tot;
    const int above = block_excl_scan256(h0 + h1, ctl + 4, tid, tot);
    if (tid == 0) ctl[3] = 0;
    __syncthreads();
    if (above < k && above + h0 + h1 >= k) ctl[3] = (above + h0 >= k) ? SEL_NB - 1 - 2 * tid : SEL_NB - 2 - 2 * tid;
    __syncthreads();
  }
  const int bstar = ctl[3];
  int cnt = 0;
#pragma unroll
  for (int u = 0; u < SEL_VPT; ++u) cnt += (tid + u * TK_NT < n) && bk[u] >= bstar;
  int total;
  int pos = block_excl_scan256(cnt, ctl + 8, tid, total);
  if (total <= SEL_CAP) {
    for (int i = total + tid; i < SEL_CAP; i += TK_NT) buf[i] = 0ull;
#pragma unroll
    for (int u = 0; u < SEL_VPT; ++u) {
      const int c = tid + u * TK_NT;
      if (c < n && bk[u] >= bstar) buf[pos++] = make_key(v[u], (uint32_t)c);
    }
    __syncthreads();
    if (total <= TK_NT)
      block_sort_desc<TK_NT, 1>(buf, tid, TK_NT);
    else
      block_sort_desc<TK_NT, SEL_CAP / TK_NT>(buf, tid, SEL_CAP);
    const int f = total < k ? total : k;
    for (int i = tid; i < k; i += TK_NT) {
      const u64 key = buf[i];
      const bool ok = i < f;
      if (D) D[(size_t)r * out_ld + i] = ok ? key_score(key) : -3.402823466e+38f;
      if (I64) I64[(size_t)r * out_ld + i] = ok ? (int64_t)key_id(key) : -1;
      if (I32) I32[(size_t)r * out_ld + i] = ok ? (int32_t)key_id(key) : -1;
    }
    return;
  }
  __syncthreads();
  StreamTopK<TK_NT> tk;
  tk.init(buf, ctl, thr, cap, k, tid);
  for (int base = 0; base < n; base += TK_NT) {
    const int c = base + tid;
    u64 key = 0ull;
    if (c < n) {
      const float x = row[c];
      const float t = fminf(fmaxf((x - lo) * scale, 0.0f), (float)(SEL_NB - 1));
      if ((int)t >= bstar) key = make_key(x, (uint32_t)c);
    }
    tk.push(key, tid);
  }
  tk.finish(D ? D + (size_t)r * out_ld : nullptr, I64 ? I64 + (size_t)r * out_ld : nullptr,
            I32 ? I32 + (size_t)r * out_ld : nullptr, tid);
}

int row_topk(const float *scores, int64_t ld, int rows, int n, int k, const int32_t *ids,
             int32_t id_base, const int32_t *vlist, const uint32_t *bitmap, int bitmap_words,
             float *D, int64_t *I64, int32_t *I32, int64_t out_ld, const uint64_t *upper_in,
             uint64_t *upper_out) {
  if (rows <= 0) return ASL_OK;
  if (k <= 0 || k > TK_MAX_K) return fail(ASL_ERR_CAPACITY, "top-k: k=%d outside 1..%d", k, TK_MAX_K);
  const int cap = topk_cap_for(k);
  if (n <= SEL_VPT * TK_NT && k <= 256 && !ids && id_base == 0 && !bitmap && !upper_in && !upper_out) {
    const size_t lds_sel = (size_t)std::max(cap, SEL_CAP) * 8 + 8 + 12 * 4 + SEL_NB * 4 + 8 * 4;
    hipLaunchKernelGGL(row_select_kernel, dim3(rows), dim3(TK_NT), lds_sel, stream(), scores, ld,
                       n, k, cap, D, I64, I32, out_ld);
    ASL_CHECK_LAUNCH();
    return ASL_OK;
  }
  const size_t lds = (size_t)cap * 8 + 16;
  if (lds > 64 * 1024)
    HIP_TRY(hipFuncSetAttribute((const void *)row_topk_kernel,
                                hipFuncAttributeMaxDynamicSharedMemorySize, (int)lds));
  hipLaunchKernelGGL(row_topk_kernel, dim3(rows), dim3(TK_NT), lds, stream(), scores, ld, n,
                     k, cap, ids, id_base, vlist, bitmap, bitmap_words, D, I64, I32, out_ld,
                     reinterpret_cast<const u64 *>(upper_in), reinterpret_cast<u64 *>(upper_out));
  ASL_CHECK_LAUNCH();
  return ASL_OK;
}

__global__ __launch_bounds__(TK_NT) void topk_merge_kernel(
    const float *__restrict__ Ds, const int64_t *__restrict__ Is, int S, int nq, int k,
    int cap, float *__restrict__ D, int64_t *__restrict__ I) {
  extern __shared__ __attribute__((aligned(16))) char smem[];
  u64 *buf = reinterpret_cast<u64 *>(smem);
  u64 *thr = buf + cap;
  int *ctl = reinterpret_cast<int *>(thr + 1);
  const int tid = threadIdx.x, q = blockIdx.x;
  StreamTopK<TK_NT> tk;
  tk.init(buf, ctl, thr, cap, k, tid);
  const int total = S * k;
  for (int base = 0; base < total; base += TK_NT) {
    const int t = base + tid;
    u64 key = 0ull;
    if (t < total) {
      const int s = t / k, i = t - s * k;
      const size_t o = ((size_t)s * nq + q) * k + i;
      const int64_t id = Is[o];
      if (id >= 0) key = make_key(Ds[o], (uint32_t)id);
    }
    tk.push(key, tid);
  }
  tk.finish(D + (size_t)q * k, I + (size_t)q * k, nullptr, tid);
}

template <int CAP, int PT, bool KEYS = false>
__global__ __launch_bounds__(HT_NT) void topk_merge_hist_kernel(
    const float *__restrict__ Ds, const int64_t *__restrict__ Is, int S, int nq, int k,
    float *__restrict__ D, int64_t *__restrict__ I, int unordered) {
  using TopK = HistTopK<CAP, HT_NT * PT>;
  extern __shared__ __attribute__((aligned(16))) char smem[];
  const int tid = threadIdx.x, q = blockIdx.x;
  TopK top;
  top.init(smem, k, nullptr, tid);
  const int kc = (k + 63) >> 6;
  const int total = kc * S * 64;
  for (int base = 0; base < total; base += HT_NT * PT) {
    top.begin_round();
    int appended = 0;
#pragma unroll
    for (int u = 0; u < PT; ++u) {
      const int v = base + u * HT_NT + tid;
      const int c = v >> 6, s = c % S, j = (c / S) * 64 + (v & 63);
      bool valid = v < total && j < k;
      float score = 0.0f;
      int64_t id = -1;
      uint32_t slot = 0;
      if (valid) {
        const size_t o = ((size_t)s * nq + q) * k + j;
        if (KEYS) {
          const u64 key = (u64)Is[o];
          valid = key != 0ull;
          score = key_score(key);
          slot = (uint32_t)key;
        } else {
          score = Ds[o];
          id = Is[o];
          valid = id >= 0;
          slot = 0xFFFFFFFFu - (uint32_t)id;
        }
      }
      const bool take = top.offer(valid, score, slot);
      appended += __popcll(__ballot(take));
    }
    top.end_round(appended);
  }
  if (unordered)
    top.finish_set(D ? D + (size_t)q * k : nullptr, I + (size_t)q * k, nullptr,
                   reinterpret_cast<u64 *>(smem + TopK::lds_bytes()));
  else
    top.finish(D ? D + (size_t)q * k : nullptr, I + (size_t)q * k, nullptr);
}

int topk_merge_keys(const int64_t *Ks, int S, int nq, int k, float *D, int64_t *I, int unordered) {
  if (nq <= 0) return ASL_OK;
  if (k <= 0 || k + 256 + 512 > 2048)
    return fail(ASL_ERR_CAPACITY, "merge_keys: k=%d outside 1..1280", k);
  const size_t lds = HistTopK<2048, HT_NT * 2>::lds_bytes() + (unordered ? (size_t)2048 * 8 : 0);
  hipLaunchKernelGGL((topk_merge_hist_kernel<2048, 2, true>), dim3(nq), dim3(HT_NT), lds, stream(),
                     (const float *)nullptr, Ks, S, nq, k, D, I, unordered);
  ASL_CHECK_LAUNCH();
  return ASL_OK;
}

int topk_merge(const float *Ds, const int64_t *Is, int S, int nq, int k, float *D, int64_t *I) {
  if (nq <= 0) return ASL_OK;
  if (k <= 0 || k > TK_MAX_K) return fail(ASL_ERR_CAPACITY, "merge: k=%d outside 1..%d", k, TK_MAX_K);
  if ((int64_t)S * k >= 2048 && k + 256 + 1024 <= 4096) {
    if (k + 256 + 512 <= 2048)
      hipLaunchKernelGGL((topk_merge_hist_kernel<2048, 2>), dim3(nq), dim3(HT_NT),
                         (HistTopK<2048, HT_NT * 2>::lds_bytes()), stream(), Ds, Is, S, nq, k, D, I, 0);
    else
      hipLaunchKernelGGL((topk_merge_hist_kernel<4096, 4>), dim3(nq), dim3(HT_NT),
                         (HistTopK<4096, HT_NT * 4>::lds_bytes()), stream(), Ds, Is, S, nq, k, D, I, 0);
    ASL_CHECK_LAUNCH();
    return ASL_OK;
  }
  const int cap = topk_cap_for(k);
  const size_t lds = (size_t)cap * 8 + 16;
  if (lds > 64 * 1024)
    HIP_TRY(hipFuncSetAttribute((const void *)topk_merge_kernel,
                                hipFuncAttributeMaxDynamicSharedMemorySize, (int)lds));
  hipLaunchKernelGGL(topk_merge_kernel, dim3(nq), dim3(TK_NT), lds, stream(), Ds, Is, S, nq, k,
                     cap, D, I);
  ASL_CHECK_LAUNCH();
  return ASL_OK;
}

__global__ void probe_bitmap_kernel(const int32_t *__restrict__ coarse_I, int nq, int nprobe,
                                    uint32_t *__restrict__ bitmap, int words) {
  const int q = blockIdx.x;
  for (int p = threadIdx.x; p < nprobe; p += blockDim.x) {
    const int l = coarse_I[(size_t)q * nprobe + p];
    if (l >= 0) atomicOr(&bitmap[(size_t)q * words + (l >> 5)], 1u << (l & 31));
  }
}

int probe_bitmap(const int32_t *coarse_I, int nq, int nprobe, uint32_t *bitmap, int words) {
  HIP_TRY(hipMemsetAsync(bitmap, 0, (size_t)nq * words * sizeof(uint32_t), stream()));
  hipLaunchKernelGGL(probe_bitmap_kernel, dim3(nq), dim3(128), 0, stream(), coarse_I, nq,
                     nprobe, bitmap, words);
  ASL_CHECK_LAUNCH();
  return ASL_OK;
}

__global__ void gather_rows_f32_kernel(const float *__restrict__ src, int64_t ld_src,
                                       const int64_t *__restrict__ rows, int64_t n, int d,
                                       float *__restrict__ dst, int64_t ld_dst) {
  const int64_t i = block_linear();
  if (i >= n) return;
  const int64_t r = rows ? rows[i] : i;
  for (int j = threadIdx.x; j < d; j += blockDim.x)
    dst[i * ld_dst + j] = src[r * ld_src + j];
}
int gather_rows_f32(const float *src, int64_t ld_src, const int64_t *rows, int64_t n, int d,
                    float *dst, int64_t ld_dst) {
  if (n <= 0) return ASL_OK;
  hipLaunchKernelGGL(gather_rows_f32_kernel, grid_2d(n), dim3(256), 0, stream(), src,
                     ld_src, rows, n, d, dst, ld_dst);
  ASL_CHECK_LAUNCH();
  return ASL_OK;
}

__global__ void gather_rows_u8_kernel(const uint8_t *__restrict__ src,
                                      const int32_t *__restrict__ rows, int64_t n, int m,
                                      uint8_t *__restrict__ dst) {
  const int64_t t = block_linear() * blockDim.x + threadIdx.x;
  if (t >= n * m) return;
  const int64_t i = t / m;
  const int j = (int)(t - i * m);
  dst[t] = src[(int64_t)rows[i] * m + j];
}
int gather_rows_u8(const uint8_t *src, const int32_t *rows, int64_t n, int m, uint8_t *dst) {
  if (n <= 0) return ASL_OK;
  hipLaunchKernelGGL(gather_rows_u8_kernel, grid_2d(cdiv(n * m, 256)), dim3(256), 0,
                     stream(), src, rows, n, m, dst);
  ASL_CHECK_LAUNCH();
  return ASL_OK;
}

__device__ __forceinline__ void build_lut_lds(const float *__restrict__ xq_row, int d,
                                              const float *__restrict__ codebooks, int m,
                                              int ksub, int dsub, float *s_q, float *s_lut,
                                              int tid) {
  for (int i = tid; i < d; i += TK_NT) s_q[i] = xq_row[i];
  __syncthreads();
  for (int c = tid; c < ksub; c += TK_NT) {
    for (int mi = 0; mi < m; ++mi) {
      const float *cb = codebooks + ((size_t)mi * ksub + c) * dsub;
      const float *qs = s_q + mi * dsub;
      float acc = 0.0f;
      for (int t = 0; t < dsub; ++t) acc = __builtin_fmaf(qs[t], cb[t], acc);
      s_lut[mi * ksub + c] = acc;
    }
  }
  __syncthreads();
}

__global__ __launch_bounds__(TK_NT) void pq_lut_kernel(const float *__restrict__ xq, int d,
                                                       const float *__restrict__ codebooks,
                                                       int m, int ksub, int dsub,
                                                       float *__restrict__ lut_out) {
  extern __shared__ __attribute__((aligned(16))) char smem[];
  float *s_lut = reinterpret_cast<float *>(smem);
  float *s_q = s_lut + m * ksub;
  const int q = blockIdx.x;
  build_lut_lds(xq + (size_t)q * d, d, codebooks, m, ksub, dsub, s_q, s_lut, threadIdx.x);
  for (int i = threadIdx.x; i < m * ksub; i += TK_NT) lut_out[(size_t)q * m * ksub + i] = s_lut[i];
}
int pq_lut(const float *xq, int nq, int d, const float *codebooks, int m, int ksub, int dsub,
           float *lut_out) {
  if (nq <= 0) return ASL_OK;
  const size_t lds = ((size_t)m * ksub + d) * 4;
  if (lds > (size_t)PQ_MAX_LDS_BYTES) return fail(ASL_ERR_CAPACITY, "pq lut: d=%d / m=%d do not fit LDS", d, m);
  if (lds > 64 * 1024)
    HIP_TRY(hipFuncSetAttribute((const void *)pq_lut_kernel,
                                hipFuncAttributeMaxDynamicSharedMemorySize, (int)lds));
  hipLaunchKernelGGL(pq_lut_kernel, dim3(nq), dim3(TK_NT), lds, stream(), xq, d, codebooks, m,
                     ksub, dsub, lut_out);
  ASL_CHECK_LAUNCH();
  return ASL_OK;
}

template <int M>
__device__ __forceinline__ float adc_score(const float *__restrict__ s_lut, int ksub,
                                           const uint32_t *__restrict__ cw, float coarse) {
  float v[M];
#pragma unroll
  for (int w = 0; w < M / 4; ++w) {
    const uint32_t word = cw[w];
#pragma unroll
    for (int b = 0; b < 4; ++b) {
      const int mi = w * 4 + b;
      v[mi] = s_lut[mi * ksub + ((word >> (8 * b)) & 0xffu)];
    }
  }
  float p[16];
#pragma unroll
  for (int j = 0; j < 16; ++j) {
    if (j < M) {
      float a = v[j];
#pragma unroll
      for (int t = j + 16; t < M; t += 16) a = a + v[t];
      p[j] = a;
    } else {
      p[j] = 0.0f;
    }
  }
#pragma unroll
  for (int j = 0; j < 8; ++j) p[j] = p[j] + p[15 - j];
#pragma unroll
  for (int j = 0; j < 4; ++j) p[j] = p[j] + p[7 - j];
#pragma unroll
  for (int j = 0; j < 2; ++j) p[j] = p[j] + p[3 - j];
  return coarse + (p[0] + p[1]);
}

template <int M>
__global__ __launch_bounds__(TK_NT) void pq_scan_kernel(
    const float *__restrict__ xq, int d, const float *__restrict__ codebooks, int ksub,
    int dsub, const float *__restrict__ coarse_D, const int32_t *__restrict__ coarse_I,
    int nprobe, const int32_t *__restrict__ list_offsets, const int32_t *__restrict__ ids,
    const uint8_t *__restrict__ codes, int k, int cap, float *__restrict__ D,
    int64_t *__restrict__ I64, int32_t *__restrict__ I32, int64_t out_ld,
    const u64 *__restrict__ upper_in, u64 *__restrict__ upper_out) {
  extern __shared__ __attribute__((aligned(16))) char smem[];
  u64 *buf = reinterpret_cast<u64 *>(smem);
  u64 *thr = buf + cap;
  int *ctl = reinterpret_cast<int *>(thr + 1);
  float *s_lut = reinterpret_cast<float *>(thr + 2);
  float *s_q = s_lut + M * ksub;
  const int tid = threadIdx.x, q = blockIdx.x;
  build_lut_lds(xq + (size_t)q * d, d, codebooks, M, ksub, dsub, s_q, s_lut, tid);
  StreamTopK<TK_NT> tk;
  tk.init(buf, ctl, thr, cap, k, tid);
  const u64 ub = upper_in ? upper_in[q] : ~0ull;
  for (int p = 0; p < nprobe; ++p) {
    const int l = coarse_I[(size_t)q * nprobe + p];
    if (l < 0) continue;
    const float coarse = coarse_D[(size_t)q * nprobe + p];
    const int start = list_offsets[l], len = list_offsets[l + 1] - start;
    for (int base = 0; base < len; base += TK_NT) {
      const int i = base + tid;
      u64 key = 0ull;
      if (i < len) {
        const uint32_t *cw = reinterpret_cast<const uint32_t *>(codes + (size_t)(start + i) * M);
        key = make_key(adc_score<M>(s_lut, ksub, cw, coarse), (uint32_t)ids[start + i]);
        if (key >= ub) key = 0ull;
      }
      tk.push(key, tid);
    }
  }
  tk.finish(D ? D + (size_t)q * out_ld : nullptr, I64 ? I64 + (size_t)q * out_ld : nullptr,
            I32 ? I32 + (size_t)q * out_ld : nullptr, tid);
  if (upper_out && tid == 0) upper_out[q] = ctl[0] >= k ? buf[k - 1] : 0ull;
}

size_t pq_scan_lds_bytes(int m, int ksub, int d, int k) {
  return (size_t)topk_cap_for(k) * 8 + 16 + ((size_t)m * ksub + d) * 4;
}

int pq_scan(const float *xq, int nq, int d, const float *codebooks, int m, int ksub, int dsub,
            const float *coarse_D, const int32_t *coarse_I, int nprobe,
            const int32_t *list_offsets, const int32_t *ids, const uint8_t *codes, int k,
            float *D, int64_t *I64, int32_t *I32, int64_t out_ld, const uint64_t *upper_in,
            uint64_t *upper_out) {
  if (nq <= 0) return ASL_OK;
  if (k <= 0 || k > TK_MAX_K) return fail(ASL_ERR_CAPACITY, "pq scan: k=%d outside 1..%d", k, TK_MAX_K);
  const auto launch = [&](auto m_const) -> int {
    constexpr int M = decltype(m_const)::value;
    const int cap = topk_cap_for(k);
    const size_t lds = pq_scan_lds_bytes(M, ksub, d, k);
    if (lds > (size_t)PQ_MAX_LDS_BYTES) return fail(ASL_ERR_CAPACITY, "pq scan: k=%d / m=%d do not fit LDS", k, M);
    if (lds > 64 * 1024)
      HIP_TRY(hipFuncSetAttribute((const void *)pq_scan_kernel<M>,
                                  hipFuncAttributeMaxDynamicSharedMemorySize, (int)lds));
    hipLaunchKernelGGL(pq_scan_kernel<M>, dim3(nq), dim3(TK_NT), lds, stream(), xq, d, codebooks,
                       ksub, dsub, coarse_D, coarse_I, nprobe, list_offsets, ids, codes, k, cap,
                       D, I64, I32, out_ld > 0 ? out_ld : (int64_t)k, reinterpret_cast<const u64 *>(upper_in),
                       reinterpret_cast<u64 *>(upper_out));
    ASL_CHECK_LAUNCH();
    return ASL_OK;
  };
  switch (m) {
    case 4: return launch(std::integral_constant<int, 4>{});
    case 8: return launch(std::integral_constant<int, 8>{});
    case 16: return launch(std::integral_constant<int, 16>{});
    case 32: return launch(std::integral_constant<int, 32>{});
    case 64: return launch(std::integral_constant<int, 64>{});
    default: return fail(ASL_ERR_INVALID, "pq scan: pq_m must be one of 4,8,16,32,64 (got %d)", m);
  }
}


__global__ void scanned_count_kernel(const int32_t *__restrict__ coarse_I, int64_t n,
                                     const int32_t *__restrict__ list_offsets,
                                     unsigned long long *__restrict__ out) {
  unsigned long long acc = 0;
  for (int64_t i = (int64_t)blockIdx.x * blockDim.x + threadIdx.x; i < n;
       i += (int64_t)gridDim.x * blockDim.x) {
    const int l = coarse_I[i];
    if (l >= 0) acc += (unsigned long long)(list_offsets[l + 1] - list_offsets[l]);
  }
  for (int off = 32; off > 0; off >>= 1) acc += __shfl_xor(acc, off);
  if ((threadIdx.x & 63) == 0 && acc) atomicAdd(out, acc);
}
int scanned_count(const int32_t *coarse_I, int64_t n, const int32_t *list_offsets,
                  unsigned long long *out_dev) {
  hipLaunchKernelGGL(scanned_count_kernel, dim3(256), dim3(256), 0, stream(), coarse_I, n,
                     list_offsets, out_dev);
  ASL_CHECK_LAUNCH();
  return ASL_OK;
}

}
```

ann_solo_amd/csrc/ivf_kernels.hpp:

```cpp
#pragma once
#include <cstdint>

#include <hip/hip_runtime.h>

namespace asl {

struct ScanPostFilter;
struct ScanRanges;
struct FlatPostings;

constexpr int TK_NT = 256;
constexpr int TK_MAX_K = 2048;
constexpr int TK_MAX_K_PASSES = 16384;
constexpr int PQ_MAX_DSUB = 32;
constexpr int PQ_MAX_LDS_BYTES = 160 * 1024;

int gemm_nt_f32(const float *A, const float *B, float *C, int M, int N, int K, int lda,
                int ldb, int ldc, const int *gate = nullptr, int gate_max = 0);

bool coarse_sparse_supported(int d, int nlist);
int coarse_sparse_cap();
int list_nonzeros(const float *xq, int nq, int d, int64_t ldq, uint2 *ent, int32_t *cnt, int *n_over);
int transpose_f32(const float *in, int rows, int cols, float *out);
int coarse_sparse(const float *xq, int nq, int d, const float *Ct, int nlist, uint2 *ent,
                  int32_t *cnt, int *n_over, int over_max, float *scores, int ld, int64_t ldq = 0);

int row_topk(const float *scores, int64_t ld, int rows, int n, int k, const int32_t *ids,
             int32_t id_base, const int32_t *vlist, const uint32_t *bitmap, int bitmap_words,
             float *D, int64_t *I64, int32_t *I32, int64_t out_ld,
             const uint64_t *upper_in = nullptr, uint64_t *upper_out = nullptr);
int topk_merge(const float *Ds, const int64_t *Is, int S, int nq, int k, float *D, int64_t *I);
int topk_merge_keys(const int64_t *Ks, int S, int nq, int k, float *D, int64_t *I, int unordered);
int probe_bitmap(const int32_t *coarse_I, int nq, int nprobe, uint32_t *bitmap, int words);
int gather_rows_f32(const float *src, int64_t ld_src, const int64_t *rows, int64_t n, int d,
                    float *dst, int64_t ld_dst);
int gather_rows_u8(const uint8_t *src, const int32_t *rows, int64_t n, int m, uint8_t *dst);
int pq_lut(const float *xq, int nq, int d, const float *codebooks, int m, int ksub, int dsub,
           float *lut_out);
int pq_scan(const float *xq, int nq, int d, const float *codebooks, int m, int ksub, int dsub,
            const float *coarse_D, const int32_t *coarse_I, int nprobe,
            const int32_t *list_offsets, const int32_t *ids, const uint8_t *codes, int k,
            float *D, int64_t *I64, int32_t *I32, int64_t out_ld = 0,
            const uint64_t *upper_in = nullptr, uint64_t *upper_out = nullptr);
size_t pq_scan_lds_bytes(int m, int ksub, int d, int k);
int scanned_count(const int32_t *coarse_I, int64_t n, const int32_t *list_offsets,
                  unsigned long long *out_dev);

int row_argmax(const float *scores, int64_t ld, int rows, int n, int32_t *out);
int centroid_update(const float *x, int64_t ld, int d, int k, const int32_t *order,
                    const int32_t *offsets, float *centroids);
int renorm_rows(float *c, int k, int d);
int l2_assign(const float *x, int64_t ld, int64_t n, int dsub, const float *cb, int ksub,
              int32_t *assign);
int residual(const float *x, const int32_t *assign, const float *centroids, int64_t n, int d,
             float *dst);
int pq_encode(const float *x, const int32_t *assign, const float *centroids,
              const float *codebooks, int64_t n, int d, int m, int ksub, int dsub,
              uint8_t *codes, bool by_residual = true);

bool pq_scan_tiled_supported(int m, int ksub, int k, int nprobe);
int pq_scan_v3(const float *xq, int nq, int d, const float *codebooks, int dsub,
               const float *coarse_D, const int32_t *coarse_I, int nprobe,
               const int32_t *list_offsets, const int32_t *tile_offsets,
               const uint8_t *codes_tiled, const int32_t *ids_tiled, int k, float *D,
               int64_t *I64, int32_t *I32, int set_mode, const uint2 *ent = nullptr,
               const int32_t *ent_cnt = nullptr,
               const int *gate = nullptr,
               const ScanPostFilter *post = nullptr,
               const ScanRanges *ranges = nullptr,
               const unsigned long long *sel = nullptr,
               const uint8_t *codes_mm = nullptr,
               uint32_t mm_plane = 0);
int mmajor_codes(const uint8_t *codes_tiled, int64_t ntiles, uint32_t plane, uint8_t *codes_mm);
int tile_selector(const int32_t *slot_ids, int64_t ntiles, const uint8_t *keep, int64_t n,
                  unsigned long long *words);
int window_ranges(const double *q_pmz, int nq, const int32_t *coarse_I, int nprobe,
                  const int32_t *list_offsets, const int32_t *tile_offsets, const float *wkey, int charge,
                  double tol, int mode, int2 *ranges, unsigned long long *acc);
int tile_codes(const uint8_t *codes, const int32_t *ids, const int32_t *dst_slot, int64_t n,
               int64_t ntiles, uint8_t *codes_tiled, int32_t *ids_tiled);


int refine_stride();
int refine_append_rows(const float *x, int64_t n, int d, int64_t row0, uint16_t *r_dim, float *r_val,
                       uint8_t *r_cnt, int *status);
int refine_topk(const float *xq, int nq, int d, const int32_t *I_in, const int64_t *I_in64, int kp,
                const uint16_t *r_dim, const float *r_val, const uint8_t *r_cnt, int64_t n_rows, int k, float *D,
                int64_t *I64, int32_t *I32);

int keys_split(const unsigned long long *K, int64_t nrows, int k, int kp, unsigned long long *head,
               int32_t *floor_out, unsigned long long *rowmin_out = nullptr);
int keys_merge(const unsigned long long *heads, int S, int nq, int kp, int k, const unsigned long long *xbuf,
               long long xcap, const unsigned long long *prev_keys, int32_t *need,
               unsigned long long *out_keys, unsigned long long *bounds, int64_t *I, float *D, int sorted);
int keys_extras(const unsigned long long *K, const int32_t *floor_in, int64_t nrows, int k,
                const unsigned long long *bounds, int nq, long long xcap, unsigned long long *xbuf,
                unsigned int *cursor, int32_t *overflow, const int32_t *rmap = nullptr,
                const unsigned long long *K3 = nullptr, int k3 = 0);
int rescan_list(const unsigned long long *bounds, const unsigned long long *rowmin, int64_t nrows, int R,
                int64_t *rowlist, int32_t *rmap, int *count, int32_t *overflow);

struct RankWindow {
  const float *key_slot = nullptr;
  const double *q_pmz = nullptr;
  double tol = 0.0;
  int mode = 0, charge = 0;
};
int rank_invert(const int32_t *slot_ids, int64_t nslots, int64_t ntotal, int32_t *inv);
int rank_slot_keys(const int32_t *slot_ids, int64_t nslots, const float *key, int64_t ntotal, float *key_slot);
int rank_flat(const FlatPostings &P, const float *xq, int nq, int64_t ntotal, const int32_t *coarse_I, int nprobe,
              const int64_t *target, const int32_t *inv, const RankWindow &win, unsigned long long *tkey,
              float *tscore, unsigned long long *counts, int want_scope);
int rank_pq(const float *xq, int nq, int d, const float *cbT, int dsub, int nlist, int64_t ntotal,
            const float *coarse_D, const int32_t *coarse_I, int nprobe, const float *coarse_all,
            const int32_t *list_offsets, const int32_t *tile_offsets, const uint8_t *codes_tiled,
            const int32_t *ids_tiled, const int64_t *target, const int32_t *inv, const RankWindow &win,
            unsigned long long *tkey, float *tscore, unsigned long long *counts, int want_scope);
int rank_finish(const unsigned long long *tkey, const float *tscore, const unsigned long long *counts, int nq,
                int64_t *rank, float *score, int64_t *scope);

}
```

ann_solo_amd/csrc/library.hpp:

```cpp
#pragma once
#include <algorithm>

#include "rescore.hpp"

struct asl_library {
  int64_t n = 0;
  uint64_t serial = 0;
  asl::DevBuf<int32_t> offsets, pcharge;
  asl::DevBuf<float> mz, intensity, pmz32;
  asl::DevBuf<uint8_t> charge, valid;
  asl::DevBuf<double> pmz;
  asl::DevBuf<uint8_t> records;
  uint32_t slot = 0;
  asl::DevBuf<float> wcol;
  bool has_valid = false;
  asl::DevBuf<uint8_t> keep, valid_eff;
  asl::DevBuf<float> wcol_eff;
  bool has_sel = false;
  uint64_t sel_gen = 0;
  const float *window_col() const { return has_sel ? wcol_eff.p : wcol.p; }
  const uint8_t *valid_col() const { return has_sel ? valid_eff.p : has_valid ? valid.p : nullptr; }
  asl::DevBuf<int32_t> group;
  bool has_group = false;
  asl::DevPeaks dev;
  asl::DevBuf<float> sorted_pmz;
  asl::DevBuf<int32_t> sorted_row;
  asl::DevBuf<float> qvec;
  asl::DevBuf<int32_t> knn, cand, lo, cnt, woff;
  asl::DevBuf<float> p_qvec[2], p_cD[2];
  asl::DevBuf<int32_t> p_cI[2], p_knn[2], p_cnt[2];
  asl::DevBuf<int32_t> p_rows[2], rows_len;
  asl::DevBuf<double> p_win[2];
  asl::DevBuf<uint2> p_ent[2];
  bool p_have_ent[2] = {false, false};
  asl::DevBuf<double> pair_score;
  asl::DevBuf<long long> best_slot;
  asl::DevBuf<int32_t> wtile, run_row, run_n, tile_n;
  asl::DevBuf<double> run_score, tile_score;
  asl::DevBuf<int> status;
  asl::RescoreScratch rs_scratch;
};

namespace asl {

inline void library_filter(const asl_library *L, PrecFilter &flt) {
  flt.meta = reinterpret_cast<const RowMeta *>(L->records.p);
  flt.meta_stride = L->slot;
  flt.wcol = L->window_col();
}
inline void batch_filter(const asl_library *L, const asl_search_params_t *P, const double *win, PrecFilter &flt) {
  flt.lib_pmz = L->pmz32.p;
  flt.valid = L->valid_col();
  library_filter(L, flt);
  flt.tol = P->precursor_tol;
  flt.mode = P->precursor_mode;
  flt.charge = P->charge;
  if (P->precursor_mode == ASL_TOL_INTERVAL) flt.interval = win;
}

struct SearchBatch {
  asl_library *L = nullptr;
  DevPeaks Q;
  const asl_search_params_t *P = nullptr;
  const double *win = nullptr;
  int n_best = 0;
  bool distinct = false;
  BatchOut out;
  size_t winners() const { return (size_t)Q.n * (size_t)std::max(n_best, 1); }
  const int32_t *group() const { return distinct ? L->group.p : nullptr; }
  const double *window_operand() const { return P->precursor_mode == ASL_TOL_INTERVAL ? win : Q.precursor_mz; }
  RescoreRequest rescore_request() const {
    return {.Q = Q, .L = L->dev, .tol = P->fragment_mz_tolerance,
            .tol_ppm = (P->allow_shift & ASL_SCORE_FRAGMENT_PPM) ? 1 : 0,
            .allow_shift = (P->allow_shift & ASL_SCORE_SHIFT) ? 1 : 0, .tie_by_row = 1,
            .n_best = n_best, .group = group(),
            .pair_score = L->pair_score.p, .best_slot = L->best_slot.p,
            .scratch = &L->rs_scratch, .status = L->status.p, .out = out};
  }
};

int window_search_device(const SearchBatch &b);

}
```

ann_solo_amd/csrc/search.hip:

```cpp
#include "index.hpp"
#include "library.hpp"

namespace asl {
int encode_device(const float *mz, const float *inten, const int32_t *offsets, int32_t n,
                  double min_bound, double bin_size, int32_t hash_len, uint32_t seed,
                  int norm, float *out);
}

using namespace asl;

static int &scan_postfilter_flag() {
  static int on = -1;
  if (on < 0) {
    const char *e = getenv("ASL_SCAN_POSTFILTER");
    on = (e && e[0] == '0') ? 0 : 1;
  }
  return on;
}

enum { ENTRY_TOPN = 1, ENTRY_DISTINCT = 2, ENTRY_KNN = 4 };
static int check_batch(const char *who, int kind, const asl_library *L, const asl_index *idx,
                       const asl_peaks_t *queries, const asl_search_params_t *P, const int64_t *knn_I, int n_best,
                       const BatchOut &out, bool *run) {
  *run = false;
  if (kind & ENTRY_TOPN) {
    if (n_best < 1 || n_best > ASL_MAX_BEST)
      return fail(ASL_ERR_INVALID, "%s: n_best must be in [1, %d]", who, ASL_MAX_BEST);
    ASL_TRY(ensure_device());
  }
  if (!L || !queries || !P || ((kind & ENTRY_KNN) && !knn_I)) return fail(ASL_ERR_INVALID, "%s: null argument", who);
  if ((kind & ENTRY_DISTINCT) && !L->has_group)
    return fail(ASL_ERR_STATE, "%s: the library has no group column (asl_library_set_groups)", who);
  if (queries->n == 0) return ASL_OK;
  if (out.pm_pairs && out.pm_stride <= 0) return fail(ASL_ERR_INVALID, "%s: pm_stride", who);
  const bool ann = !(kind & ENTRY_KNN) && P->use_ann;
  if (ann && !idx) return fail(ASL_ERR_INVALID, "%s: use_ann needs an index", who);
  if ((ann || (kind & ENTRY_KNN)) && P->k <= 0) return fail(ASL_ERR_INVALID, "%s: k must be positive", who);
  if (P->precursor_mode == ASL_TOL_INTERVAL && !P->precursor_window)
    return fail(ASL_ERR_INVALID, "%s: precursor_mode ASL_TOL_INTERVAL needs precursor_window ([nq, 2] doubles)", who);
  ScoreFlags sf;
  ASL_TRY(decode_score_flags(P->allow_shift, who, sf));
  *run = true;
  return ASL_OK;
}

struct BatchScan {
  IndexSearch rq;
  IndexWindow w;
  IndexPostFilter pf;
};
static void batch_scan(BatchScan &s, const SearchBatch &b, const asl_index *idx, int nprobe, const float *xq,
                       int64_t *I64, int32_t *I32, int32_t *row_len, const float *pre_D = nullptr,
                       const int32_t *pre_I = nullptr, const uint2 *pre_ent = nullptr,
                       const int32_t *pre_cnt = nullptr) {
  const asl_library *L = b.L;
  const asl_search_params_t *P = b.P;
  const bool as_set = I64 == nullptr;
  s.rq = {.nq = b.Q.n, .xq = xq, .k = P->k, .nprobe = nprobe, .I64 = I64, .I32 = I32, .pre_D = pre_D, .pre_I = pre_I,
          .pre_ent = pre_ent, .pre_cnt = pre_cnt, .rows = as_set ? ROWS_SET : ROWS_ORDERED};
  s.rq.serial = L->serial;
  s.rq.gen = L->sel_gen;
  if (L->has_sel) {
    s.rq.sel_keep = L->keep.p;
    s.rq.sel_n = L->n;
  }
  if (window_mode(idx)) {
    s.w = {.q_pmz = b.window_operand(), .row_len = as_set ? row_len : nullptr, .tol = P->precursor_tol,
           .mode = P->precursor_mode, .charge = P->charge};
    s.rq.win = &s.w;
  } else if (as_set && scan_postfilter_flag() == 1) {
    s.pf = {.payload = L->window_col(), .n = L->n, .q_pmz = b.window_operand(), .count = row_len,
            .tol = P->precursor_tol, .mode = P->precursor_mode, .charge = P->charge};
    s.rq.post = &s.pf;
  }
}

static RescoreRequest rows_request(const SearchBatch &b, CandList cand) {
  cand.stride = b.P->k;
  cand.total_slots = (int64_t)b.Q.n * b.P->k;
  RescoreRequest rq = b.rescore_request();
  rq.cand = cand;
  batch_filter(b.L, b.P, b.win, rq.filter);
  return rq;
}

static BatchOut row_outputs(int32_t *row, double *score, int32_t *n_cand, int32_t *count, uint32_t *pairs, int32_t stride,
                            int32_t *hist = nullptr) {
  return {.best_row = row, .best_score = score, .n_cand = n_cand, .pm_count = count, .pm_pairs = pairs, .pm_stride = stride,
          .score_hist = hist};
}

static int search_batch_sync(asl_library *L, asl_index *idx, const asl_peaks_t *queries,
                             const asl_search_params_t *P, int n_best, bool distinct, const BatchOut &out,
                             const int64_t *knn_in, int64_t *knn_out) {
  const int nq = queries->n, k = P->k;
  ASL_TRY(ensure_device());
  PeaksStage Q;
  ASL_TRY(Q.init(queries));
  In<double> dwin;
  if (P->precursor_mode == ASL_TOL_INTERVAL) ASL_TRY(dwin.init(P->precursor_window, (size_t)nq * 2));
  SearchBatch b{.L = L, .Q = Q.dev, .P = P, .win = dwin.d, .n_best = n_best, .distinct = distinct};
  BatchOutStage o;
  ASL_TRY(o.init(out, (size_t)nq, b.winners()));
  b.out = o.dev;
  In<int64_t> knn;
  Out<int64_t> o_knn;
  ASL_TRY(L->best_slot.reserve(b.winners()));
  ASL_TRY(L->status.reserve(1));
  if (knn_in) {
    ASL_TRY(knn.init(knn_in, (size_t)nq * k));
    ASL_TRY(L->pair_score.reserve((size_t)nq * k));
    ASL_TRY(rescore_device(rows_request(b, {.rows64 = knn.d})));
  } else if (P->use_ann) {
    const int d = idx->d;
    ASL_TRY(o_knn.init(knn_out, (size_t)nq * k));
    ASL_TRY(L->qvec.reserve((size_t)nq * d));
    ASL_TRY(L->knn.reserve((size_t)nq * k));
    ASL_TRY(L->pair_score.reserve((size_t)nq * k));
    ASL_TRY(L->rows_len.reserve((size_t)nq));
    if (window_mode(idx))
      ASL_TRY(index_window_prepare(idx, L->serial, L->sel_gen, L->window_col(), L->n, nq, P->nprobe));
    ASL_TRY(encode_device(Q.dev.mz, Q.dev.intensity, Q.dev.offsets, nq, P->min_bound, P->bin_size,
                          d, P->hash_seed, 1, L->qvec.p));
    BatchScan s;
    batch_scan(s, b, idx, P->nprobe, L->qvec.p, o_knn.d, L->knn.p, L->rows_len.p);
    ASL_TRY(index_search_device(idx, s.rq));
    ASL_TRY(rescore_device(rows_request(b, {.rows32 = L->knn.p,
                                            .row_counts = s.rq.rows_filtered ? L->rows_len.p : nullptr})));
  } else {
    ASL_TRY(window_search_device(b));
  }
  ASL_TRY(o.finish());
  ASL_TRY(o_knn.finish());
  return rescore_check_status(L->status.p);
}

static int search_batch_pipelined(asl_library *L, asl_index *idx, const asl_peaks_t *queries,
                                  const asl_search_params_t *P, const BatchOut &out, int64_t *knn_I) {
  Pipeline &pp = pipeline();
  struct InCall {
    Pipeline &p;
    explicit InCall(Pipeline &q) : p(q) { p.in_call = true; }
    ~InCall() { p.in_call = false; }
  } guard(pp);
  const int nq = queries->n, k = P->k, d = idx->d;
  const bool winflat = idx->kind == ASL_INDEX_WINFLAT;
  const int nprobe = winflat ? 1 : index_nprobe(idx, P->nprobe);
  PeaksStage Q;
  ASL_TRY(Q.init(queries));
  const int par = pp.parity;
  ASL_TRY(index_prepare(idx));
  if (window_mode(idx))
    ASL_TRY(index_window_prepare(idx, L->serial, L->sel_gen, L->window_col(), L->n, nq, nprobe));
  ASL_TRY(L->p_qvec[par].reserve((size_t)nq * d));
  ASL_TRY(L->p_cD[par].reserve((size_t)nq * nprobe));
  ASL_TRY(L->p_cI[par].reserve((size_t)nq * nprobe));
  ASL_TRY(L->p_knn[par].reserve((size_t)nq * k));
  ASL_TRY(L->p_ent[par].reserve((size_t)nq * 64));
  ASL_TRY(L->p_cnt[par].reserve((size_t)nq));
  ASL_TRY(L->p_rows[par].reserve((size_t)nq));
  ASL_TRY(L->pair_score.reserve((size_t)nq * k));
  ASL_TRY(L->best_slot.reserve((size_t)nq));
  const double *dwin = nullptr;
  if (P->precursor_mode == ASL_TOL_INTERVAL) {
    dwin = P->precursor_window;
    if (!is_device_ptr(dwin)) {
      ASL_TRY(L->p_win[par].reserve((size_t)nq * 2));
      if (pp.resc_recorded[par]) HIP_TRY(hipStreamWaitEvent(stream(), pp.ev_resc[par], 0));
      HIP_TRY(hipMemcpyAsync(L->p_win[par].p, dwin, (size_t)nq * 16, hipMemcpyHostToDevice, stream()));
      HIP_TRY(hipStreamSynchronize(stream()));
      dwin = L->p_win[par].p;
    }
  }
  pp.parity ^= 1;
  HIP_TRY(hipEventRecord(pp.ev_in, stream()));
  HIP_TRY(hipStreamWaitEvent(pp.A, pp.ev_in, 0));
  HIP_TRY(hipStreamWaitEvent(pp.B, pp.ev_in, 0));
  HIP_TRY(hipStreamWaitEvent(pp.C, pp.ev_in, 0));
  pp.inflight = true;
  const SearchBatch b{.L = L, .Q = Q.dev, .P = P, .win = dwin, .out = out};
  BatchScan s;
  {
    StreamScope on_a(pp.A);
    if (pp.scan_recorded[par]) HIP_TRY(hipStreamWaitEvent(pp.A, pp.ev_scan[par], 0));
    ASL_TRY(encode_device(Q.dev.mz, Q.dev.intensity, Q.dev.offsets, nq, P->min_bound, P->bin_size,
                          d, P->hash_seed, 1, L->p_qvec[par].p));
    if (winflat)
      L->p_have_ent[par] = false;
    else
      ASL_TRY(coarse_search(idx, L->p_qvec[par].p, nq, nprobe, L->p_cD[par].p, L->p_cI[par].p,
                                  L->p_ent[par].p, L->p_cnt[par].p, &L->p_have_ent[par]));
    HIP_TRY(hipEventRecord(pp.ev_front[par], pp.A));
  }
  {
    StreamScope on_b(pp.B);
    HIP_TRY(hipStreamWaitEvent(pp.B, pp.ev_front[par], 0));
    if (pp.resc_recorded[par]) HIP_TRY(hipStreamWaitEvent(pp.B, pp.ev_resc[par], 0));
    const bool ent = L->p_have_ent[par];
    batch_scan(s, b, idx, nprobe, L->p_qvec[par].p, knn_I, L->p_knn[par].p, L->p_rows[par].p,
               winflat ? nullptr : L->p_cD[par].p, winflat ? nullptr : L->p_cI[par].p,
               ent ? L->p_ent[par].p : nullptr, ent ? L->p_cnt[par].p : nullptr);
    ASL_TRY(index_search_device(idx, s.rq));
    HIP_TRY(hipEventRecord(pp.ev_scan[par], pp.B));
    pp.scan_recorded[par] = true;
  }
  {
    hipStream_t sc = pp.streams == 3 ? pp.C : pp.B;
    StreamScope on_c(sc);
    HIP_TRY(hipStreamWaitEvent(sc, pp.ev_scan[par], 0));
    RescoreRequest rq = rows_request(b, {.rows32 = L->p_knn[par].p,
                                         .row_counts = s.rq.rows_filtered ? L->p_rows[par].p : nullptr});
    rq.status = pp.status;
    rq.clear_status = false;
    ASL_TRY(rescore_device(rq));
    HIP_TRY(hipEventRecord(pp.ev_resc[par], sc));
    pp.resc_recorded[par] = true;
  }
  return ASL_OK;
}

extern "C" {

int asl_set_scan_postfilter(int on) {
  clear_error();
  int &f = scan_postfilter_flag();
  const int prev = f;
  f = on ? 1 : 0;
  return prev;
}

int asl_search_batch(asl_library_t *L, asl_index_t *idx, const asl_peaks_t *queries,
                     const asl_search_params_t *P, int32_t *best_row, double *best_score,
                     int32_t *n_cand, int32_t *pm_count, uint32_t *pm_pairs, int32_t pm_stride,
                     int64_t *knn_I) {
  clear_error();
  const BatchOut out = row_outputs(best_row, best_score, n_cand, pm_count, pm_pairs, pm_stride);
  bool run;
  ASL_TRY(check_batch("search_batch", 0, L, idx, queries, P, nullptr, 0, out, &run));
  if (!run) return ASL_OK;
  {
    Pipeline &pp = pipeline();
    auto dev_or_null = [](const void *p) { return !p || is_device_ptr(p); };
    if (pp.on && P->use_ann && (index_nprobe(idx, P->nprobe) > 0 || idx->kind == ASL_INDEX_WINFLAT) &&
        queries->n_peaks > 0 &&
        peaks_on_device(queries) &&
        is_device_ptr(best_row) && is_device_ptr(best_score) && dev_or_null(n_cand) &&
        dev_or_null(pm_count) && dev_or_null(pm_pairs) && dev_or_null(knn_I)) {
      pp.in_call = true;
      const int rc = ensure_device();
      pp.in_call = false;
      ASL_TRY(rc);
      return search_batch_pipelined(L, idx, queries, P, out, knn_I);
    }
  }
  return search_batch_sync(L, idx, queries, P, 0, false, out, nullptr, knn_I);
}

static int checked_batch_sync(const char *who, int kind, asl_library_t *L, asl_index_t *idx, const asl_peaks_t *queries,
                              const asl_search_params_t *P, int n_best, const BatchOut &out, const int64_t *knn_in,
                              int64_t *knn_out) {
  clear_error();
  bool run;
  ASL_TRY(check_batch(who, kind, L, idx, queries, P, knn_in, n_best, out, &run));
  if (!run) return ASL_OK;
  return search_batch_sync(L, idx, queries, P, n_best, (kind & ENTRY_DISTINCT) != 0, out, knn_in, knn_out);
}

int asl_search_batch_topn(asl_library_t *L, asl_index_t *idx, const asl_peaks_t *queries,
                          const asl_search_params_t *P, int32_t n_best, int32_t *best_row, double *best_score,
                          int32_t *n_cand, int32_t *pm_count, uint32_t *pm_pairs, int32_t pm_stride,
                          int64_t *knn_I) {
  return checked_batch_sync("search_batch_topn", ENTRY_TOPN, L, idx, queries, P, n_best,
                            row_outputs(best_row, best_score, n_cand, pm_count, pm_pairs, pm_stride), nullptr, knn_I);
}

int asl_search_batch_topn_distinct(asl_library_t *L, asl_index_t *idx, const asl_peaks_t *queries,
                                   const asl_search_params_t *P, int32_t n_best, int32_t *best_row,
                                   double *best_score, int32_t *n_cand, int32_t *pm_count, uint32_t *pm_pairs,
                                   int32_t pm_stride, int64_t *knn_I) {
  return checked_batch_sync("search_batch_topn_distinct", ENTRY_TOPN | ENTRY_DISTINCT, L, idx, queries, P, n_best,
                            row_outputs(best_row, best_score, n_cand, pm_count, pm_pairs, pm_stride), nullptr, knn_I);
}

int asl_rescore_knn(asl_library_t *L, const asl_peaks_t *queries, const asl_search_params_t *P,
                    const int64_t *knn_I, int32_t *best_row, double *best_score,
                    int32_t *n_cand, int32_t *pm_count, uint32_t *pm_pairs, int32_t pm_stride) {
  return checked_batch_sync("rescore_knn", ENTRY_KNN, L, nullptr, queries, P, 0,
                            row_outputs(best_row, best_score, n_cand, pm_count, pm_pairs, pm_stride), knn_I, nullptr);
}

int asl_rescore_knn_topn(asl_library_t *L, const asl_peaks_t *queries, const asl_search_params_t *P,
                         const int64_t *knn_I, int32_t n_best, int32_t *best_row, double *best_score,
                         int32_t *n_cand, int32_t *pm_count, uint32_t *pm_pairs, int32_t pm_stride) {
  return checked_batch_sync("rescore_knn_topn", ENTRY_KNN | ENTRY_TOPN, L, nullptr, queries, P, n_best,
                            row_outputs(best_row, best_score, n_cand, pm_count, pm_pairs, pm_stride), knn_I, nullptr);
}

int asl_rescore_knn_topn_distinct(asl_library_t *L, const asl_peaks_t *queries, const asl_search_params_t *P,
                                  const int64_t *knn_I, int32_t n_best, int32_t *best_row, double *best_score,
                                  int32_t *n_cand, int32_t *pm_count, uint32_t *pm_pairs, int32_t pm_stride) {
  return checked_batch_sync("rescore_knn_topn_distinct", ENTRY_KNN | ENTRY_TOPN | ENTRY_DISTINCT, L, nullptr, queries, P,
                            n_best, row_outputs(best_row, best_score, n_cand, pm_count, pm_pairs, pm_stride), knn_I,
                            nullptr);
}

int asl_search_batch_topn_hist(asl_library_t *L, asl_index_t *idx, const asl_peaks_t *queries,
                               const asl_search_params_t *P, int32_t n_best, int32_t distinct, int32_t *best_row,
                               double *best_score, int32_t *n_cand, int32_t *pm_count, uint32_t *pm_pairs,
                               int32_t pm_stride, int64_t *knn_I, int32_t *score_hist) {
  return checked_batch_sync("search_batch_topn_hist", ENTRY_TOPN | (distinct ? ENTRY_DISTINCT : 0), L, idx, queries, P,
                            n_best, row_outputs(best_row, best_score, n_cand, pm_count, pm_pairs, pm_stride, score_hist),
                            nullptr, knn_I);
}

int asl_rescore_knn_topn_hist(asl_library_t *L, const asl_peaks_t *queries, const asl_search_params_t *P,
                              const int64_t *knn_I, int32_t n_best, int32_t distinct, int32_t *best_row,
                              double *best_score, int32_t *n_cand, int32_t *pm_count, uint32_t *pm_pairs,
                              int32_t pm_stride, int32_t *score_hist) {
  return checked_batch_sync("rescore_knn_topn_hist", ENTRY_KNN | ENTRY_TOPN | (distinct ? ENTRY_DISTINCT : 0), L, nullptr,
                            queries, P, n_best,
                            row_outputs(best_row, best_score, n_cand, pm_count, pm_pairs, pm_stride, score_hist), knn_I,
                            nullptr);
}

}
```

ann_solo_amd/csrc/topk.hpp:

```cpp
#pragma once
#include <hip/hip_runtime.h>

#include <cstdint>

namespace asl {

typedef unsigned long long u64;

__device__ __forceinline__ uint32_t f2ord(float f) {
  const uint32_t u = __float_as_uint(f);
  return (u & 0x80000000u) ? ~u : (u | 0x80000000u);
}
__device__ __forceinline__ float ord2f(uint32_t o) {
  const uint32_t u = (o & 0x80000000u) ? (o & 0x7fffffffu) : ~o;
  return __uint_as_float(u);
}
__device__ __forceinline__ u64 make_key(float score, uint32_t id) {
  return ((u64)f2ord(score) << 32) | (u64)(0xFFFFFFFFu - id);
}
__device__ __forceinline__ float key_score(u64 k) { return ord2f((uint32_t)(k >> 32)); }
__device__ __forceinline__ uint32_t key_id(u64 k) { return 0xFFFFFFFFu - (uint32_t)k; }

template <int NT>
__device__ __forceinline__ void bitonic_sort_desc(u64 *buf, int n, int tid) {
  for (int k = 2; k <= n; k <<= 1) {
    for (int j = k >> 1; j > 0; j >>= 1) {
      for (int t = tid; t < (n >> 1); t += NT) {
        const int i = ((t & ~(j - 1)) << 1) | (t & (j - 1));
        const int l = i | j;
        const u64 a = buf[i], b = buf[l];
        const bool desc = (i & k) == 0;
        if (desc ? (a < b) : (a > b)) {
          buf[i] = b;
          buf[l] = a;
        }
      }
      __syncthreads();
    }
  }
}

template <int NT, int CAP>
__device__ __forceinline__ void bitonic_sort_desc_ct(u64 *buf, int tid) {
  constexpr int PER = CAP / (2 * NT);
  static_assert(PER >= 1, "CAP must be at least 2*NT");
#pragma nounroll
  for (int k = 2; k <= CAP; k <<= 1) {
#pragma nounroll
    for (int j = k >> 1; j > 0; j >>= 1) {
      u64 a[PER], b[PER];
      int ia[PER];
#pragma unroll
      for (int u = 0; u < PER; ++u) {
        const int t = tid + u * NT;
        ia[u] = ((t & ~(j - 1)) << 1) | (t & (j - 1));
        a[u] = buf[ia[u]];
        b[u] = buf[ia[u] | j];
      }
#pragma unroll
      for (int u = 0; u < PER; ++u) {
        const bool desc = (ia[u] & k) == 0;
        if (desc ? (a[u] < b[u]) : (a[u] > b[u])) {
          buf[ia[u]] = b[u];
          buf[ia[u] | j] = a[u];
        }
      }
      __syncthreads();
    }
  }
}

__device__ __forceinline__ void wave_lds_sync() {
  __builtin_amdgcn_fence(__ATOMIC_RELEASE, "wavefront");
  __builtin_amdgcn_wave_barrier();
  __builtin_amdgcn_fence(__ATOMIC_ACQUIRE, "wavefront");
}

template <int CTRL>
__device__ __forceinline__ u64 dpp_u64(u64 v) {
  const int lo = __builtin_amdgcn_update_dpp(0, (int)(uint32_t)v, CTRL, 0xf, 0xf, false);
  const int hi = __builtin_amdgcn_update_dpp(0, (int)(uint32_t)(v >> 32), CTRL, 0xf, 0xf, false);
  return ((u64)(uint32_t)hi << 32) | (u64)(uint32_t)lo;
}

template <int NT, int P>
__device__ __forceinline__ void block_sort_desc(u64 *buf, int tid, int n_out) {
  u64 x[P];
#pragma unroll
  for (int r = 0; r < P; ++r) x[r] = buf[r * NT + tid];
  __syncthreads();
#pragma unroll
  for (int k = 2; k <= P; k <<= 1) {
#pragma unroll
    for (int j = k >> 1; j > 0; j >>= 1) {
#pragma unroll
      for (int r = 0; r < P; ++r) {
        if ((r & j) == 0) {
          const int l = r | j;
          const bool desc = (k < P) ? ((r & k) == 0) : ((tid & 1) == 0);
          const bool lt = x[r] < x[l];
          const bool sw = (lt == desc);
          const u64 a = sw ? x[l] : x[r], b = sw ? x[r] : x[l];
          x[r] = a;
          x[l] = b;
        }
      }
    }
  }
#pragma nounroll
  for (int k = 2 * P; k <= NT * P; k <<= 1) {
    const bool desc = (tid & (k / P)) == 0;
#pragma nounroll
    for (int j = k >> 1; j >= P; j >>= 1) {
      const int jj = j / P;
      const bool keep_max = (((tid & jj) == 0) == desc);
      u64 y[P];
      if (jj >= 64) {
#pragma unroll
        for (int r = 0; r < P; ++r) buf[r * NT + tid] = x[r];
        __syncthreads();
#pragma unroll
        for (int r = 0; r < P; ++r) y[r] = buf[r * NT + (tid ^ jj)];
        __syncthreads();
      } else if (jj == 1) {
#pragma unroll
        for (int r = 0; r < P; ++r) y[r] = dpp_u64<0xB1>(x[r]);
      } else if (jj == 2) {
#pragma unroll
        for (int r = 0; r < P; ++r) y[r] = dpp_u64<0x4E>(x[r]);
      } else {
#pragma unroll
        for (int r = 0; r < P; ++r) y[r] = __shfl_xor(x[r], jj, 64);
      }
#pragma unroll
      for (int r = 0; r < P; ++r) {
        const bool gt = y[r] > x[r];
        x[r] = (gt == keep_max) ? y[r] : x[r];
      }
    }
#pragma unroll
    for (int j = P >> 1; j > 0; j >>= 1) {
#pragma unroll
      for (int r = 0; r < P; ++r) {
        if ((r & j) == 0) {
          const int l = r | j;
          const bool lt = x[r] < x[l];
          const bool sw = (lt == desc);
          const u64 a = sw ? x[l] : x[r], b = sw ? x[r] : x[l];
          x[r] = a;
          x[l] = b;
        }
      }
    }
  }
  __syncthreads();
  if (tid * P < n_out) {
#pragma unroll
    for (int r = 0; r < P; ++r) buf[tid * P + r] = x[r];
  }
  __syncthreads();
}

template <int NT, int CAP = 0>
struct StreamTopK {
  u64 *buf;
  int *ctl;
  u64 *thr;
  int cap, k;
  bool force_rt = false;
  const int32_t *slot_ids = nullptr;
  int conv_from = 0;
  bool emit_keys = false;

  __device__ __forceinline__ void init(u64 *b, int *c, u64 *t, int cap_, int k_, int tid) {
    buf = b;
    ctl = c;
    thr = t;
    cap = cap_;
    k = k_;
    for (int i = tid; i < cap; i += NT) buf[i] = 0ull;
    if (tid == 0) {
      ctl[0] = 0;
      *thr = 0ull;
    }
    __syncthreads();
  }

  __device__ __forceinline__ void push(u64 key, int tid) {
    __syncthreads();
    if (key > *thr) {
      const int s = atomicAdd(&ctl[0], 1);
      buf[s] = key;
    }
    __syncthreads();
    if (ctl[0] > cap - NT) flush(tid);
  }

  __device__ __forceinline__ int flush(int tid) {
    const int f = ctl[0];
    __syncthreads();
    if (slot_ids) {
      if constexpr (CAP > 0) {
        constexpr int PERC = CAP / NT;
        u64 kk[PERC];
        int32_t idv[PERC];
#pragma unroll
        for (int u = 0; u < PERC; ++u) {
          const int i = conv_from + tid + u * NT;
          kk[u] = i < f ? buf[i] : 0ull;
        }
#pragma unroll
        for (int u = 0; u < PERC; ++u) {
          const int i = conv_from + tid + u * NT;
          idv[u] = (i < f && kk[u] != 0ull) ? slot_ids[(uint32_t)kk[u]] : -1;
        }
#pragma unroll
        for (int u = 0; u < PERC; ++u) {
          const int i = conv_from + tid + u * NT;
          if (i < f)
            buf[i] = idv[u] >= 0 ? ((kk[u] & 0xFFFFFFFF00000000ull) |
                                    (u64)(0xFFFFFFFFu - (uint32_t)idv[u])) : 0ull;
        }
      } else {
        for (int i = conv_from + tid; i < f; i += NT) {
          const u64 key = buf[i];
          const int32_t id = key != 0ull ? slot_ids[(uint32_t)key] : -1;
          buf[i] = id >= 0 ? ((key & 0xFFFFFFFF00000000ull) | (u64)(0xFFFFFFFFu - (uint32_t)id)) : 0ull;
        }
      }
    }
    for (int i = f + tid; i < cap; i += NT) buf[i] = 0ull;
    __syncthreads();
    if (CAP > 0 && !force_rt)
      block_sort_desc<NT, (CAP > 0 ? CAP / NT : 2)>(buf, tid, k);
    else
      bitonic_sort_desc<NT>(buf, cap, tid);
    const int nf = f < k ? f : k;
    conv_from = nf;
    if (tid == 0) {
      ctl[0] = nf;
      *thr = (nf == k) ? buf[k - 1] : 0ull;
    }
    __syncthreads();
    return nf;
  }

  __device__ __forceinline__ void finish(float *D, int64_t *I, int32_t *I32, int tid) {
    __syncthreads();
    flush(tid);
    const int f = ctl[0];
    for (int i = tid; i < k; i += NT) {
      const u64 key = buf[i];
      const bool ok = i < f;
      if (D) D[i] = ok ? key_score(key) : -3.402823466e+38f;
      if (I) I[i] = emit_keys ? (ok ? (int64_t)key : 0) : (ok ? (int64_t)key_id(key) : -1);
      if (I32) I32[i] = ok ? (int32_t)key_id(key) : -1;
    }
  }
};

inline int topk_cap_for(int k) {
  int cap = 1024;
  while (cap < 4 * k) cap <<= 1;
  return cap;
}

}
```

Before: 3.164 million query spectra/s.

## Fuse query sparse-entry listing into encode and use wave-level row select

The encode kernel gains a variant that writes both the dense normalized query vector and its sparse nonzero entry list, so the coarse sparse scorer can skip its separate list_nonzeros launch and memset when the lists are already prepared. Coarse search and the IVF search paths thread these precomputed lists through, gated by an environment switch that is on by default. Separately, the per-row top-k selection kernel is replaced by a wave-per-row design using DPP min/max reductions, per-wave histograms and a wave-local sort, which removes block-wide barriers and processes several rows per block. This adds more code paths and capacity conditions that must match for the fused path to be taken.

```diff
diff --git a/ann_solo_amd/csrc/coarse_sparse.hip b/ann_solo_amd/csrc/coarse_sparse.hip
--- a/ann_solo_amd/csrc/coarse_sparse.hip
+++ b/ann_solo_amd/csrc/coarse_sparse.hip
@@ -192,13 +192,15 @@
 }
 
 int coarse_sparse(const float *xq, int nq, int d, const float *Ct, int nlist, uint2 *ent,
-                  int32_t *cnt, int *n_over, int over_max, float *scores, int ld, int64_t ldq) {
+                  int32_t *cnt, int *n_over, int over_max, float *scores, int ld, int64_t ldq, bool lists_ready) {
   if (ldq <= 0) ldq = d;
   if (nq <= 0) return ASL_OK;
-  HIP_TRY(hipMemsetAsync(n_over, 0, sizeof(int), stream()));
-  hipLaunchKernelGGL(list_nonzeros_kernel, dim3((unsigned)cdiv(nq, 4)), dim3(256), 0, stream(), xq,
-                     nq, d, ldq, ent, cnt, n_over);
-  ASL_CHECK_LAUNCH();
+  if (!lists_ready) {
+    HIP_TRY(hipMemsetAsync(n_over, 0, sizeof(int), stream()));
+    hipLaunchKernelGGL(list_nonzeros_kernel, dim3((unsigned)cdiv(nq, 4)), dim3(256), 0, stream(), xq,
+                       nq, d, ldq, ent, cnt, n_over);
+    ASL_CHECK_LAUNCH();
+  }
   const int tiles = (int)cdiv(nlist, CS_TL);
   int parts = std::max(1, std::min((512 + tiles - 1) / tiles, (nq + 4 * CS_NW - 1) / (4 * CS_NW)));
   const size_t lds = (size_t)d * CS_TL * 4;
diff --git a/ann_solo_amd/csrc/encode.hip b/ann_solo_amd/csrc/encode.hip
--- a/ann_solo_amd/csrc/encode.hip
+++ b/ann_solo_amd/csrc/encode.hip
@@ -133,7 +133,7 @@
 constexpr int QE_CAP = 64;
 constexpr int QE_DIM_SHIFT = 7;
 
-template <bool ENTRIES>
+template <bool ENTRIES, bool DENSE_TOO = false>
 __global__ __launch_bounds__(64 * ENC_WAVES) void encode_kernel(
     const float *__restrict__ mz, const float *__restrict__ inten,
     const int32_t *__restrict__ offsets, int32_t n, double min_bound, double bin_size,
@@ -185,10 +185,10 @@
     }
     nrm = __builtin_sqrtf(acc);
   }
-  if (!ENTRIES) {
+  if (!ENTRIES || DENSE_TOO) {
     float *row = out + (size_t)spec * hash_len;
     for (int i = lane; i < hash_len; i += 64) row[i] = norm ? vec[i] / nrm : vec[i];
-    return;
+    if (!ENTRIES) return;
   }
   uint2 *row = ent + (size_t)spec * QE_CAP;
   int have = 0;
@@ -211,17 +211,16 @@
   }
 }
 
-template <bool ENTRIES>
-static int encode_launch(const float *mz, const float *inten, const int32_t *offsets, int32_t n,
+template <typename K>
+static int encode_launch(K kern, const float *mz, const float *inten, const int32_t *offsets, int32_t n,
                          double min_bound, double bin_size, int32_t hash_len, uint32_t seed, int norm,
                          float *out, uint2 *ent, int32_t *ent_cnt, int *n_over) {
   size_t lds = (size_t)ENC_WAVES * hash_len * sizeof(float);
   if (lds > 160 * 1024) return fail(ASL_ERR_CAPACITY, "encode: hash_len %d too large for LDS", hash_len);
   dim3 grid((unsigned)cdiv(n, ENC_WAVES));
   if (lds > 64 * 1024)
-    HIP_TRY(hipFuncSetAttribute((const void *)encode_kernel<ENTRIES>,
-                                hipFuncAttributeMaxDynamicSharedMemorySize, (int)lds));
-  hipLaunchKernelGGL(encode_kernel<ENTRIES>, grid, dim3(64 * ENC_WAVES), lds, stream(), mz, inten,
+    HIP_TRY(hipFuncSetAttribute((const void *)kern, hipFuncAttributeMaxDynamicSharedMemorySize, (int)lds));
+  hipLaunchKernelGGL(kern, grid, dim3(64 * ENC_WAVES), lds, stream(), mz, inten,
                      offsets, n, min_bound, bin_size, hash_len, seed, norm, out, ent, ent_cnt, n_over);
   ASL_CHECK_LAUNCH();
   return ASL_OK;
@@ -232,7 +231,7 @@
                   int norm, float *out) {
   if (n == 0) return ASL_OK;
   ProfScope ps("encode");
-  return encode_launch<false>(mz, inten, offsets, n, min_bound, bin_size, hash_len, seed, norm, out,
+  return encode_launch(encode_kernel<false>, mz, inten, offsets, n, min_bound, bin_size, hash_len, seed, norm, out,
                               nullptr, nullptr, nullptr);
 }
 
@@ -241,8 +240,17 @@
                           uint2 *ent, int32_t *cnt, int *n_over) {
   if (n == 0) return ASL_OK;
   ProfScope ps("encode");
-  return encode_launch<true>(mz, inten, offsets, n, min_bound, bin_size, hash_len, seed, norm, nullptr,
-                             ent, cnt, n_over);
+  return encode_launch(encode_kernel<true>, mz, inten, offsets, n, min_bound, bin_size, hash_len, seed, norm,
+                       nullptr, ent, cnt, n_over);
+}
+
+int encode_both_device(const float *mz, const float *inten, const int32_t *offsets, int32_t n,
+                       double min_bound, double bin_size, int32_t hash_len, uint32_t seed, int norm,
+                       float *out, uint2 *ent, int32_t *cnt, int *n_over) {
+  if (n == 0) return ASL_OK;
+  ProfScope ps("encode");
+  return encode_launch(encode_kernel<true, true>, mz, inten, offsets, n, min_bound, bin_size, hash_len, seed, norm, out,
+                       ent, cnt, n_over);
 }
 
 }
diff --git a/ann_solo_amd/csrc/index.hpp b/ann_solo_amd/csrc/index.hpp
--- a/ann_solo_amd/csrc/index.hpp
+++ b/ann_solo_amd/csrc/index.hpp
@@ -32,6 +32,7 @@
   const int32_t *pre_I = nullptr;
   const uint2 *pre_ent = nullptr;
   const int32_t *pre_cnt = nullptr;
+  int *pre_over = nullptr;
   const int *gate = nullptr;
   int rows = ROWS_ORDERED;
   const IndexPostFilter *post = nullptr;
@@ -165,11 +166,14 @@
 int index_nprobe(const asl_index *ix, int nprobe);
 int index_prepare(asl_index *ix);
 int coarse_search(asl_index *ix, const float *xq, int nq, int nprobe, float *out_D, int32_t *out_I, uint2 *ent_out,
-                  int32_t *cnt_out, bool *have_ent);
+                  int32_t *cnt_out, bool *have_ent, const uint2 *pre_ent = nullptr, const int32_t *pre_cnt = nullptr,
+                  int *pre_over = nullptr);
+int coarse_lists_begin(asl_index *ix, int nq, int **over);
 int index_window_prepare(asl_index *ix, uint64_t serial, uint64_t gen, const float *key, int64_t n, int nq,
                          int nprobe);
 int index_refine_k(const asl_index *ix);
-int coarse_scores_all(asl_index *ix, const float *xq, int m, float *scores, uint2 *ent = nullptr, int32_t *cnt = nullptr);
+int coarse_scores_all(asl_index *ix, const float *xq, int m, float *scores, uint2 *ent = nullptr, int32_t *cnt = nullptr,
+                      int *ready_over = nullptr);
 int index_codebooks_transposed(asl_index *ix);
 int index_codes_mmajor(asl_index *ix);
 int index_zero_coarse(asl_index *ix, size_t n, const float **zeros);
diff --git a/ann_solo_amd/csrc/index_search.hip b/ann_solo_amd/csrc/index_search.hip
--- a/ann_solo_amd/csrc/index_search.hip
+++ b/ann_solo_amd/csrc/index_search.hip
@@ -12,7 +12,7 @@
   return ASL_OK;
 }
 
-int coarse_scores_all(asl_index *ix, const float *xq, int m, float *scores, uint2 *ent, int32_t *cnt) {
+int coarse_scores_all(asl_index *ix, const float *xq, int m, float *scores, uint2 *ent, int32_t *cnt, int *ready_over) {
   const int nlist = ix->nlist, d = ix->d;
   const bool sparse = ix->scan_variant == 0 && coarse_sparse_supported(d, nlist);
   const int over_max = m / 64;
@@ -22,13 +22,14 @@
     ASL_TRY(ix->cs_cnt.reserve((size_t)m));
     ASL_TRY(ix->cs_over.reserve(1));
     ASL_TRY(coarse_sparse(xq, m, d, ix->centroids_t.p, nlist, ent ? ent : ix->cs_ent.p, cnt ? cnt : ix->cs_cnt.p,
-                          ix->cs_over.p, over_max, scores, nlist));
-  }
-  return gemm_nt_f32(xq, ix->centroids.p, scores, m, nlist, d, d, d, nlist, sparse ? ix->cs_over.p : nullptr, over_max);
+                          ready_over ? ready_over : ix->cs_over.p, over_max, scores, nlist, 0, ready_over != nullptr));
+  }
+  return gemm_nt_f32(xq, ix->centroids.p, scores, m, nlist, d, d, d, nlist,
+                     sparse ? (ready_over ? ready_over : ix->cs_over.p) : nullptr, over_max);
 }
 
 int coarse_search(asl_index *ix, const float *xq, int nq, int nprobe, float *out_D, int32_t *out_I, uint2 *ent_out,
-                  int32_t *cnt_out, bool *have_ent) {
+                  int32_t *cnt_out, bool *have_ent, const uint2 *pre_ent, const int32_t *pre_cnt, int *pre_over) {
   const int nlist = ix->nlist, d = ix->d;
   if (have_ent) *have_ent = false;
   if (!out_D) {
@@ -40,12 +41,17 @@
   int rows = (int)std::min<int64_t>(nq, std::max<int64_t>(1, (int64_t)(SCORE_CHUNK_BYTES / ((size_t)nlist * 4))));
   ASL_TRY(ix->ws_scores.reserve((size_t)rows * nlist));
   const bool sparse = ix->scan_variant == 0 && coarse_sparse_supported(d, nlist);
+  const bool ready = sparse && pre_ent && pre_cnt && pre_over && nq <= rows && coarse_sparse_cap() == 64;
   for (int r0 = 0; r0 < nq; r0 += rows) {
     const int m = std::min(rows, nq - r0);
     {
       ProfScope ps("coarse_gemm");
-      ASL_TRY(coarse_scores_all(ix, xq + (size_t)r0 * d, m, ix->ws_scores.p, ent_out ? ent_out + (size_t)r0 * 64 : nullptr,
-                                cnt_out ? cnt_out + (size_t)r0 : nullptr));
+      if (ready)
+        ASL_TRY(coarse_scores_all(ix, xq, m, ix->ws_scores.p, const_cast<uint2 *>(pre_ent),
+                                  const_cast<int32_t *>(pre_cnt), pre_over));
+      else
+        ASL_TRY(coarse_scores_all(ix, xq + (size_t)r0 * d, m, ix->ws_scores.p, ent_out ? ent_out + (size_t)r0 * 64 : nullptr,
+                                  cnt_out ? cnt_out + (size_t)r0 : nullptr));
     }
     {
       ProfScope ps("coarse_select");
@@ -54,6 +60,23 @@
     }
   }
   if (have_ent) *have_ent = sparse && coarse_sparse_cap() == 64 && ((ent_out && cnt_out) || nq <= rows);
+  return ASL_OK;
+}
+
+static bool coarse_lists_enabled() {
+  const char *e = getenv("ASL_COARSE_LISTS");
+  return !(e && e[0] == '0');
+}
+
+int coarse_lists_begin(asl_index *ix, int nq, int **over) {
+  *over = nullptr;
+  if (!coarse_lists_enabled() || nq <= 0 || ix->nlist <= 0) return ASL_OK;
+  if (ix->kind != ASL_INDEX_IVFFLAT && ix->kind != ASL_INDEX_IVFPQ) return ASL_OK;
+  if (!(ix->scan_variant == 0 && coarse_sparse_supported(ix->d, ix->nlist)) || coarse_sparse_cap() != 64) return ASL_OK;
+  if ((size_t)nq > SCORE_CHUNK_BYTES / ((size_t)ix->nlist * 4)) return ASL_OK;
+  ASL_TRY(ix->cs_over.reserve(1));
+  HIP_TRY(hipMemsetAsync(ix->cs_over.p, 0, sizeof(int), stream()));
+  *over = ix->cs_over.p;
   return ASL_OK;
 }
 
@@ -141,9 +164,11 @@
       return fail(ASL_ERR_INVALID, "selector: %lld flags for %lld vectors", (long long)rq.sel_n, (long long)ix->ntotal);
   }
   if (rq.nq <= 0) return ASL_OK;
-  if (rq.pre_ent && (!rq.pre_cnt || !rq.pre_I || (!rq.xq && !rq.pre_D) || ix->kind == ASL_INDEX_FLAT))
-    return fail(ASL_ERR_STATE, "entry-list search: needs the counts, the caller's probe lists (with their scores when "
-                               "no dense rows are given) and an IVF index");
+  if (rq.pre_ent && (!rq.pre_cnt || ix->kind == ASL_INDEX_FLAT ||
+                     (rq.pre_I ? (!rq.xq && !rq.pre_D) : (!rq.xq || !rq.pre_over || rq.pre_D != nullptr))))
+    return fail(ASL_ERR_STATE, "entry-list search: needs the counts, an IVF index, and the caller's probe lists (with "
+                               "their scores when no dense rows are given) or the dense rows and the lists' count "
+                               "of dense rows");
   if (!rq.xq && !rq.pre_ent) return fail(ASL_ERR_INVALID, "search: null queries");
   if (rq.gate && (!rq.pre_I || ix->kind == ASL_INDEX_FLAT))
     return fail(ASL_ERR_STATE, "gated search: needs the caller's probe lists and an IVF index");
@@ -273,7 +298,9 @@
 static int search_ivfflat(asl_index *ix, IndexSearch &rq, const SearchPlan &pl) {
   const int nq = rq.nq, nprobe = pl.nprobe;
   bool own_ent = false;
-  if (!rq.pre_I) ASL_TRY(coarse_search(ix, rq.xq, nq, nprobe, nullptr, nullptr, nullptr, nullptr, &own_ent));
+  if (!rq.pre_I)
+    ASL_TRY(coarse_search(ix, rq.xq, nq, nprobe, nullptr, nullptr, nullptr, nullptr, &own_ent, rq.pre_ent, rq.pre_cnt,
+                          rq.pre_over));
   const int32_t *cI = rq.pre_I ? rq.pre_I : ix->coarse_I.p;
   if (!pl.use_inv) return search_gemm_topk(ix, rq, cI, nprobe);
   const uint2 *q_ent;
@@ -396,7 +423,9 @@
 static int search_ivfpq(asl_index *ix, IndexSearch &rq, const SearchPlan &pl) {
   const int nq = rq.nq, nprobe = pl.nprobe;
   bool own_ent = false;
-  if (!rq.pre_D) ASL_TRY(coarse_search(ix, rq.xq, nq, nprobe, nullptr, nullptr, nullptr, nullptr, &own_ent));
+  if (!rq.pre_D)
+    ASL_TRY(coarse_search(ix, rq.xq, nq, nprobe, nullptr, nullptr, nullptr, nullptr, &own_ent, rq.pre_ent, rq.pre_cnt,
+                          rq.pre_over));
   const float *cD = rq.pre_D ? rq.pre_D : ix->coarse_D.p;
   const int32_t *cI = rq.pre_D ? rq.pre_I : ix->coarse_I.p;
   if (!ix->by_residual) ASL_TRY(index_zero_coarse(ix, (size_t)nq * nprobe, &cD));
diff --git a/ann_solo_amd/csrc/ivf_kernels.hip b/ann_solo_amd/csrc/ivf_kernels.hip
--- a/ann_solo_amd/csrc/ivf_kernels.hip
+++ b/ann_solo_amd/csrc/ivf_kernels.hip
@@ -45,106 +45,229 @@
 }
 
 constexpr int SEL_VPT = 16, SEL_CAP = 512, SEL_NB = 512;
-
-__global__ __launch_bounds__(TK_NT) void row_select_kernel(
-    const float *__restrict__ scores, int64_t ld, int n, int k, int cap, float *__restrict__ D,
+constexpr int SEL_WAVES = TK_NT / 64;
+
+template <int CTRL>
+__device__ __forceinline__ float dpp_f32(float v) {
+  return __int_as_float(__builtin_amdgcn_update_dpp(0, __float_as_int(v), CTRL, 0xf, 0xf, false));
+}
+
+__device__ __forceinline__ void wave_minmax(float &lo, float &hi) {
+  lo = fminf(lo, dpp_f32<0xB1>(lo));
+  hi = fmaxf(hi, dpp_f32<0xB1>(hi));
+  lo = fminf(lo, dpp_f32<0x4E>(lo));
+  hi = fmaxf(hi, dpp_f32<0x4E>(hi));
+  lo = fminf(lo, dpp_f32<0x141>(lo));
+  hi = fmaxf(hi, dpp_f32<0x141>(hi));
+  lo = fminf(lo, dpp_f32<0x140>(lo));
+  hi = fmaxf(hi, dpp_f32<0x140>(hi));
+  float l4[4], h4[4];
+#pragma unroll
+  for (int i = 0; i < 4; ++i) {
+    l4[i] = __int_as_float(__builtin_amdgcn_readlane(__float_as_int(lo), 16 * i));
+    h4[i] = __int_as_float(__builtin_amdgcn_readlane(__float_as_int(hi), 16 * i));
+  }
+  lo = fminf(fminf(l4[0], l4[1]), fminf(l4[2], l4[3]));
+  hi = fmaxf(fmaxf(h4[0], h4[1]), fmaxf(h4[2], h4[3]));
+}
+
+struct SelThr {
+  int b, ge, gt;
+};
+
+__device__ __forceinline__ SelThr wave_threshold(const int *hist, int lane, int need) {
+  const int first = SEL_NB - 8 - 8 * lane;
+  const int4 a = *reinterpret_cast<const int4 *>(hist + first);
+  const int4 c = *reinterpret_cast<const int4 *>(hist + first + 4);
+  const int h[8] = {a.x, a.y, a.z, a.w, c.x, c.y, c.z, c.w};
+  const int s = ((h[0] + h[1]) + (h[2] + h[3])) + ((h[4] + h[5]) + (h[6] + h[7]));
+  int incl = s;
+#pragma unroll
+  for (int o = 1; o < 64; o <<= 1) {
+    const int t = __shfl_up(incl, o, 64);
+    if (lane >= o) incl += t;
+  }
+  int acc = incl - s, b = 0, ge = 0, gt = 0;
+  const bool mine = acc < need && incl >= need;
+  bool done = false;
+#pragma unroll
+  for (int i = 7; i >= 0; --i) {
+    const int nxt = acc + h[i];
+    if (!done && nxt >= need) {
+      b = first + i;
+      ge = nxt;
+      gt = acc;
+      done = true;
+    }
+    acc = nxt;
+  }
+  const u64 m = __ballot(mine);
+  SelThr t;
+  if (m == 0ull) {
+    t.b = 0;
+    t.ge = __builtin_amdgcn_readlane(incl, 63);
+    t.gt = 0;
+  } else {
+    const int src = __ffsll((long long)m) - 1;
+    t.b = __builtin_amdgcn_readlane(b, src);
+    t.ge = __builtin_amdgcn_readlane(ge, src);
+    t.gt = __builtin_amdgcn_readlane(gt, src);
+  }
+  return t;
+}
+
+__device__ __forceinline__ void wave_hist_clear(int *hist, int lane) {
+  wave_lds_sync();
+  reinterpret_cast<int4 *>(hist)[2 * lane] = make_int4(0, 0, 0, 0);
+  reinterpret_cast<int4 *>(hist)[2 * lane + 1] = make_int4(0, 0, 0, 0);
+  wave_lds_sync();
+}
+
+template <int CH, bool FULL>
+__global__ __launch_bounds__(TK_NT, 4) void wave_select_kernel(
+    const float *__restrict__ scores, int64_t ld, int rows, int n, int k, float *__restrict__ D,
     int64_t *__restrict__ I64, int32_t *__restrict__ I32, int64_t out_ld) {
-  extern __shared__ __attribute__((aligned(16))) char smem[];
-  u64 *buf = reinterpret_cast<u64 *>(smem);
-  const int nkeys = cap > SEL_CAP ? cap : SEL_CAP;
-  u64 *thr = buf + nkeys;
-  int *ctl = reinterpret_cast<int *>(thr + 1);
-  int *hist = ctl + 12;
-  float *red = reinterpret_cast<float *>(hist + SEL_NB);
-  const int tid = threadIdx.x, lane = tid & 63, wave = tid >> 6, r = blockIdx.x;
+  constexpr int NV = CH * 4;
+  __shared__ __attribute__((aligned(16))) int s_hist[SEL_WAVES][SEL_NB];
+  __shared__ __attribute__((aligned(16))) u64 s_buf[SEL_WAVES][SEL_CAP];
+  const int lane = threadIdx.x & 63;
+  const int wave = __builtin_amdgcn_readfirstlane(threadIdx.x >> 6);
+  const int r = blockIdx.x * SEL_WAVES + wave;
+  if (r >= rows) return;
+  int *hist = s_hist[wave];
+  u64 *buf = s_buf[wave];
   const float *row = scores + (size_t)r * ld;
-  float v[SEL_VPT];
+  const int c0 = lane * 4;
+  const bool wide = FULL || (reinterpret_cast<uintptr_t>(row) & 15) == 0;
+  auto chunk = [&](int u, float *x) {
+    const int c = c0 + u * 256;
+    if (FULL || (wide && c + 3 < n)) {
+      const float4 t = *reinterpret_cast<const float4 *>(row + c);
+      x[0] = t.x, x[1] = t.y, x[2] = t.z, x[3] = t.w;
+    } else {
+#pragma unroll
+      for (int e = 0; e < 4; ++e) x[e] = c + e < n ? row[c + e] : 0.0f;
+    }
+  };
+  auto col = [&](int j) { return c0 + (j >> 2) * 256 + (j & 3); };
+  auto valid = [&](int c) { return FULL || c < n; };
+
+  float v[NV];
+#pragma unroll
+  for (int u = 0; u < CH; ++u) chunk(u, v + 4 * u);
   float lo = 3.402823466e+38f, hi = -3.402823466e+38f;
 #pragma unroll
-  for (int u = 0; u < SEL_VPT; ++u) {
-    const int c = tid + u * TK_NT;
-    v[u] = c < n ? row[c] : 0.0f;
-    if (c < n) {
-      lo = fminf(lo, v[u]);
-      hi = fmaxf(hi, v[u]);
-    }
-  }
-#pragma unroll
-  for (int o = 32; o > 0; o >>= 1) {
-    lo = fminf(lo, __shfl_xor(lo, o, 64));
-    hi = fmaxf(hi, __shfl_xor(hi, o, 64));
-  }
-  if (lane == 0) {
-    red[wave] = lo;
-    red[4 + wave] = hi;
-  }
-  for (int i = tid; i < SEL_NB; i += TK_NT) hist[i] = 0;
-  __syncthreads();
-  lo = fminf(fminf(red[0], red[1]), fminf(red[2], red[3]));
-  hi = fmaxf(fmaxf(red[4], red[5]), fmaxf(red[6], red[7]));
+  for (int j = 0; j < NV; ++j)
+    if (valid(col(j))) {
+      lo = fminf(lo, v[j]);
+      hi = fmaxf(hi, v[j]);
+    }
+  wave_minmax(lo, hi);
   const float scale = hi > lo ? (float)(SEL_NB - 1) / (hi - lo) : 0.0f;
-  int bk[SEL_VPT];
-#pragma unroll
-  for (int u = 0; u < SEL_VPT; ++u) {
-    const int c = tid + u * TK_NT;
-    float t = (v[u] - lo) * scale;
-    t = fminf(fmaxf(t, 0.0f), (float)(SEL_NB - 1));
-    bk[u] = (int)t;
-    if (c < n) atomicAdd(&hist[bk[u]], 1);
-  }
-  __syncthreads();
-  {
-    const int h0 = hist[SEL_NB - 1 - 2 * tid], h1 = hist[SEL_NB - 2 - 2 * tid];
-    int tot;
-    const int above = block_excl_scan256(h0 + h1, ctl + 4, tid, tot);
-    if (tid == 0) ctl[3] = 0;
-    __syncthreads();
-    if (above < k && above + h0 + h1 >= k) ctl[3] = (above + h0 >= k) ? SEL_NB - 1 - 2 * tid : SEL_NB - 2 - 2 * tid;
-    __syncthreads();
-  }
-  const int bstar = ctl[3];
-  int cnt = 0;
-#pragma unroll
-  for (int u = 0; u < SEL_VPT; ++u) cnt += (tid + u * TK_NT < n) && bk[u] >= bstar;
-  int total;
-  int pos = block_excl_scan256(cnt, ctl + 8, tid, total);
-  if (total <= SEL_CAP) {
-    for (int i = total + tid; i < SEL_CAP; i += TK_NT) buf[i] = 0ull;
-#pragma unroll
-    for (int u = 0; u < SEL_VPT; ++u) {
-      const int c = tid + u * TK_NT;
-      if (c < n && bk[u] >= bstar) buf[pos++] = make_key(v[u], (uint32_t)c);
-    }
-    __syncthreads();
-    if (total <= TK_NT)
-      block_sort_desc<TK_NT, 1>(buf, tid, TK_NT);
-    else
-      block_sort_desc<TK_NT, SEL_CAP / TK_NT>(buf, tid, SEL_CAP);
-    const int f = total < k ? total : k;
-    for (int i = tid; i < k; i += TK_NT) {
-      const u64 key = buf[i];
-      const bool ok = i < f;
-      if (D) D[(size_t)r * out_ld + i] = ok ? key_score(key) : -3.402823466e+38f;
-      if (I64) I64[(size_t)r * out_ld + i] = ok ? (int64_t)key_id(key) : -1;
-      if (I32) I32[(size_t)r * out_ld + i] = ok ? (int32_t)key_id(key) : -1;
-    }
-    return;
-  }
-  __syncthreads();
-  StreamTopK<TK_NT> tk;
-  tk.init(buf, ctl, thr, cap, k, tid);
-  for (int base = 0; base < n; base += TK_NT) {
-    const int c = base + tid;
-    u64 key = 0ull;
-    if (c < n) {
-      const float x = row[c];
-      const float t = fminf(fmaxf((x - lo) * scale, 0.0f), (float)(SEL_NB - 1));
-      if ((int)t >= bstar) key = make_key(x, (uint32_t)c);
-    }
-    tk.push(key, tid);
-  }
-  tk.finish(D ? D + (size_t)r * out_ld : nullptr, I64 ? I64 + (size_t)r * out_ld : nullptr,
-            I32 ? I32 + (size_t)r * out_ld : nullptr, tid);
+  float plo = lo, pscale = scale;
+  auto bucket = [&](float x) {
+    const float t = fminf(fmaxf((x - plo) * pscale, 0.0f), (float)(SEL_NB - 1));
+    return (int)t;
+  };
+  wave_hist_clear(hist, lane);
+#pragma unroll
+  for (int j = 0; j < NV; ++j)
+    if (valid(col(j))) atomicAdd(&hist[bucket(v[j])], 1);
+  wave_lds_sync();
+  const SelThr th = wave_threshold(hist, lane, k);
+
+  int total = 0;
+  auto append = [&](float x, int c, bool sel) {
+    const u64 m = __ballot(sel);
+    const int pos = __builtin_amdgcn_mbcnt_hi((uint32_t)(m >> 32), __builtin_amdgcn_mbcnt_lo((uint32_t)m, total));
+    if (sel && pos < SEL_CAP) buf[pos] = make_key(x, (uint32_t)c);
+    total += __popcll(m);
+  };
+  asm volatile("" : "+v"(plo), "+v"(pscale));
+  if (th.ge <= SEL_CAP) {
+#pragma unroll
+    for (int j = 0; j < NV; ++j) append(v[j], col(j), valid(col(j)) && bucket(v[j]) >= th.b);
+  } else {
+    int in = th.gt;
+    u64 klo = ~0ull, khi = 0ull;
+#pragma nounroll
+    for (int u = 0; u < CH; ++u) {
+      float x[4];
+      chunk(u, x);
+#pragma unroll
+      for (int e = 0; e < 4; ++e) {
+        const int c = c0 + u * 256 + e;
+        const u64 key = make_key(x[e], (uint32_t)c);
+        if (valid(c) && bucket(x[e]) == th.b) {
+          klo = key < klo ? key : klo;
+          khi = key > khi ? key : khi;
+        }
+      }
+    }
+#pragma unroll
+    for (int o = 32; o > 0; o >>= 1) {
+      const u64 a = __shfl_xor(klo, o, 64), c = __shfl_xor(khi, o, 64);
+      klo = a < klo ? a : klo;
+      khi = c > khi ? c : khi;
+    }
+    u64 kthr;
+#pragma nounroll
+    for (;;) {
+      const u64 range = khi - klo;
+      const int sh = (range >> 9) ? 64 - 9 - __clzll((long long)range) : 0;
+      wave_hist_clear(hist, lane);
+#pragma nounroll
+      for (int u = 0; u < CH; ++u) {
+        float x[4];
+        chunk(u, x);
+#pragma unroll
+        for (int e = 0; e < 4; ++e) {
+          const int c = c0 + u * 256 + e;
+          const u64 key = make_key(x[e], (uint32_t)c);
+          if (valid(c) && key >= klo && key <= khi) atomicAdd(&hist[(int)((key - klo) >> sh)], 1);
+        }
+      }
+      wave_lds_sync();
+      const SelThr t2 = wave_threshold(hist, lane, k - in);
+      kthr = klo + ((u64)t2.b << sh);
+      if (in + t2.ge <= SEL_CAP) break;
+      in += t2.gt;
+      klo = kthr;
+      const u64 top = kthr + ((1ull << sh) - 1ull);
+      khi = top < khi ? top : khi;
+      wave_lds_sync();
+    }
+#pragma nounroll
+    for (int u = 0; u < CH; ++u) {
+      float x[4];
+      chunk(u, x);
+#pragma unroll
+      for (int e = 0; e < 4; ++e) {
+        const int c = c0 + u * 256 + e;
+        append(x[e], c, valid(c) && make_key(x[e], (uint32_t)c) >= kthr);
+      }
+    }
+    total = total < SEL_CAP ? total : SEL_CAP;
+  }
+  const int cap = total <= 64 ? 64 : total <= 128 ? 128 : total <= 256 ? 256 : SEL_CAP;
+  for (int i = total + lane; i < cap; i += 64) buf[i] = 0ull;
+  wave_lds_sync();
+  if (cap == 64)
+    block_sort_desc<64, 1, true>(buf, lane, k);
+  else if (cap == 128)
+    block_sort_desc<64, 2, true>(buf, lane, k);
+  else if (cap == 256)
+    block_sort_desc<64, 4, true>(buf, lane, k);
+  else
+    block_sort_desc<64, 8, true>(buf, lane, k);
+  const int f = total < k ? total : k;
+  for (int i = lane; i < k; i += 64) {
+    const u64 key = buf[i];
+    const bool ok = i < f;
+    if (D) D[(size_t)r * out_ld + i] = ok ? key_score(key) : -3.402823466e+38f;
+    if (I64) I64[(size_t)r * out_ld + i] = ok ? (int64_t)key_id(key) : -1;
+    if (I32) I32[(size_t)r * out_ld + i] = ok ? (int32_t)key_id(key) : -1;
+  }
 }
 
 int row_topk(const float *scores, int64_t ld, int rows, int n, int k, const int32_t *ids,
@@ -155,9 +278,17 @@
   if (k <= 0 || k > TK_MAX_K) return fail(ASL_ERR_CAPACITY, "top-k: k=%d outside 1..%d", k, TK_MAX_K);
   const int cap = topk_cap_for(k);
   if (n <= SEL_VPT * TK_NT && k <= 256 && !ids && id_base == 0 && !bitmap && !upper_in && !upper_out) {
-    const size_t lds_sel = (size_t)std::max(cap, SEL_CAP) * 8 + 8 + 12 * 4 + SEL_NB * 4 + 8 * 4;
-    hipLaunchKernelGGL(row_select_kernel, dim3(rows), dim3(TK_NT), lds_sel, stream(), scores, ld,
-                       n, k, cap, D, I64, I32, out_ld);
+    const dim3 grid((rows + SEL_WAVES - 1) / SEL_WAVES), block(TK_NT);
+    const bool full = n == SEL_VPT * TK_NT && ld % 4 == 0 && (reinterpret_cast<uintptr_t>(scores) & 15) == 0;
+    if (full)
+      hipLaunchKernelGGL((wave_select_kernel<SEL_VPT, true>), grid, block, 0, stream(), scores, ld, rows,
+                         n, k, D, I64, I32, out_ld);
+    else if (n <= SEL_VPT / 4 * TK_NT)
+      hipLaunchKernelGGL((wave_select_kernel<SEL_VPT / 4, false>), grid, block, 0, stream(), scores, ld,
+                         rows, n, k, D, I64, I32, out_ld);
+    else
+      hipLaunchKernelGGL((wave_select_kernel<SEL_VPT, false>), grid, block, 0, stream(), scores, ld, rows,
+                         n, k, D, I64, I32, out_ld);
     ASL_CHECK_LAUNCH();
     return ASL_OK;
   }
diff --git a/ann_solo_amd/csrc/ivf_kernels.hpp b/ann_solo_amd/csrc/ivf_kernels.hpp
--- a/ann_solo_amd/csrc/ivf_kernels.hpp
+++ b/ann_solo_amd/csrc/ivf_kernels.hpp
@@ -23,7 +23,8 @@
 int list_nonzeros(const float *xq, int nq, int d, int64_t ldq, uint2 *ent, int32_t *cnt, int *n_over);
 int transpose_f32(const float *in, int rows, int cols, float *out);
 int coarse_sparse(const float *xq, int nq, int d, const float *Ct, int nlist, uint2 *ent,
-                  int32_t *cnt, int *n_over, int over_max, float *scores, int ld, int64_t ldq = 0);
+                  int32_t *cnt, int *n_over, int over_max, float *scores, int ld, int64_t ldq = 0,
+                  bool lists_ready = false);
 
 int row_topk(const float *scores, int64_t ld, int rows, int n, int k, const int32_t *ids,
              int32_t id_base, const int32_t *vlist, const uint32_t *bitmap, int bitmap_words,
diff --git a/ann_solo_amd/csrc/library.hpp b/ann_solo_amd/csrc/library.hpp
--- a/ann_solo_amd/csrc/library.hpp
+++ b/ann_solo_amd/csrc/library.hpp
@@ -26,6 +26,8 @@
   asl::DevBuf<float> sorted_pmz;
   asl::DevBuf<int32_t> sorted_row;
   asl::DevBuf<float> qvec;
+  asl::DevBuf<uint2> q_ent;
+  asl::DevBuf<int32_t> q_cnt;
   asl::DevBuf<int32_t> knn, cand, lo, cnt, woff;
   asl::DevBuf<float> p_qvec[2], p_cD[2];
   asl::DevBuf<int32_t> p_cI[2], p_knn[2], p_cnt[2];
diff --git a/ann_solo_amd/csrc/search.hip b/ann_solo_amd/csrc/search.hip
--- a/ann_solo_amd/csrc/search.hip
+++ b/ann_solo_amd/csrc/search.hip
@@ -5,6 +5,9 @@
 int encode_device(const float *mz, const float *inten, const int32_t *offsets, int32_t n,
                   double min_bound, double bin_size, int32_t hash_len, uint32_t seed,
                   int norm, float *out);
+int encode_both_device(const float *mz, const float *inten, const int32_t *offsets, int32_t n,
+                       double min_bound, double bin_size, int32_t hash_len, uint32_t seed, int norm,
+                       float *out, uint2 *ent, int32_t *cnt, int *n_over);
 }
 
 using namespace asl;
@@ -52,12 +55,12 @@
 static void batch_scan(BatchScan &s, const SearchBatch &b, const asl_index *idx, int nprobe, const float *xq,
                        int64_t *I64, int32_t *I32, int32_t *row_len, const float *pre_D = nullptr,
                        const int32_t *pre_I = nullptr, const uint2 *pre_ent = nullptr,
-                       const int32_t *pre_cnt = nullptr) {
+                       const int32_t *pre_cnt = nullptr, int *pre_over = nullptr) {
   const asl_library *L = b.L;
   const asl_search_params_t *P = b.P;
   const bool as_set = I64 == nullptr;
   s.rq = {.nq = b.Q.n, .xq = xq, .k = P->k, .nprobe = nprobe, .I64 = I64, .I32 = I32, .pre_D = pre_D, .pre_I = pre_I,
-          .pre_ent = pre_ent, .pre_cnt = pre_cnt, .rows = as_set ? ROWS_SET : ROWS_ORDERED};
+          .pre_ent = pre_ent, .pre_cnt = pre_cnt, .pre_over = pre_over, .rows = as_set ? ROWS_SET : ROWS_ORDERED};
   s.rq.serial = L->serial;
   s.rq.gen = L->sel_gen;
   if (L->has_sel) {
@@ -120,10 +123,20 @@
     ASL_TRY(L->rows_len.reserve((size_t)nq));
     if (window_mode(idx))
       ASL_TRY(index_window_prepare(idx, L->serial, L->sel_gen, L->window_col(), L->n, nq, P->nprobe));
-    ASL_TRY(encode_device(Q.dev.mz, Q.dev.intensity, Q.dev.offsets, nq, P->min_bound, P->bin_size,
-                          d, P->hash_seed, 1, L->qvec.p));
+    int *over = nullptr;
+    ASL_TRY(coarse_lists_begin(idx, nq, &over));
+    if (over) {
+      ASL_TRY(L->q_ent.reserve((size_t)nq * 64));
+      ASL_TRY(L->q_cnt.reserve((size_t)nq));
+      ASL_TRY(encode_both_device(Q.dev.mz, Q.dev.intensity, Q.dev.offsets, nq, P->min_bound, P->bin_size,
+                                 d, P->hash_seed, 1, L->qvec.p, L->q_ent.p, L->q_cnt.p, over));
+    } else {
+      ASL_TRY(encode_device(Q.dev.mz, Q.dev.intensity, Q.dev.offsets, nq, P->min_bound, P->bin_size,
+                            d, P->hash_seed, 1, L->qvec.p));
+    }
     BatchScan s;
-    batch_scan(s, b, idx, P->nprobe, L->qvec.p, o_knn.d, L->knn.p, L->rows_len.p);
+    batch_scan(s, b, idx, P->nprobe, L->qvec.p, o_knn.d, L->knn.p, L->rows_len.p, nullptr, nullptr,
+               over ? L->q_ent.p : nullptr, over ? L->q_cnt.p : nullptr, over);
     ASL_TRY(index_search_device(idx, s.rq));
     ASL_TRY(rescore_device(rows_request(b, {.rows32 = L->knn.p,
                                             .row_counts = s.rq.rows_filtered ? L->rows_len.p : nullptr})));
@@ -183,13 +196,20 @@
   {
     StreamScope on_a(pp.A);
     if (pp.scan_recorded[par]) HIP_TRY(hipStreamWaitEvent(pp.A, pp.ev_scan[par], 0));
-    ASL_TRY(encode_device(Q.dev.mz, Q.dev.intensity, Q.dev.offsets, nq, P->min_bound, P->bin_size,
-                          d, P->hash_seed, 1, L->p_qvec[par].p));
+    int *over = nullptr;
+    if (!winflat) ASL_TRY(coarse_lists_begin(idx, nq, &over));
+    if (over)
+      ASL_TRY(encode_both_device(Q.dev.mz, Q.dev.intensity, Q.dev.offsets, nq, P->min_bound, P->bin_size,
+                                 d, P->hash_seed, 1, L->p_qvec[par].p, L->p_ent[par].p, L->p_cnt[par].p, over));
+    else
+      ASL_TRY(encode_device(Q.dev.mz, Q.dev.intensity, Q.dev.offsets, nq, P->min_bound, P->bin_size,
+                            d, P->hash_seed, 1, L->p_qvec[par].p));
     if (winflat)
       L->p_have_ent[par] = false;
     else
       ASL_TRY(coarse_search(idx, L->p_qvec[par].p, nq, nprobe, L->p_cD[par].p, L->p_cI[par].p,
-                                  L->p_ent[par].p, L->p_cnt[par].p, &L->p_have_ent[par]));
+                            L->p_ent[par].p, L->p_cnt[par].p, &L->p_have_ent[par],
+                            over ? L->p_ent[par].p : nullptr, over ? L->p_cnt[par].p : nullptr, over));
     HIP_TRY(hipEventRecord(pp.ev_front[par], pp.A));
   }
   {
diff --git a/ann_solo_amd/csrc/topk.hpp b/ann_solo_amd/csrc/topk.hpp
--- a/ann_solo_amd/csrc/topk.hpp
+++ b/ann_solo_amd/csrc/topk.hpp
@@ -83,12 +83,13 @@
   return ((u64)(uint32_t)hi << 32) | (u64)(uint32_t)lo;
 }
 
-template <int NT, int P>
+template <int NT, int P, bool WAVE = false>
 __device__ __forceinline__ void block_sort_desc(u64 *buf, int tid, int n_out) {
+  static_assert(!WAVE || NT == 64, "a wave-local sort has 64 threads");
   u64 x[P];
 #pragma unroll
   for (int r = 0; r < P; ++r) x[r] = buf[r * NT + tid];
-  __syncthreads();
+  if constexpr (WAVE) wave_lds_sync(); else __syncthreads();
 #pragma unroll
   for (int k = 2; k <= P; k <<= 1) {
 #pragma unroll
@@ -115,7 +116,7 @@
       const int jj = j / P;
       const bool keep_max = (((tid & jj) == 0) == desc);
       u64 y[P];
-      if (jj >= 64) {
+      if (!WAVE && jj >= 64) {
 #pragma unroll
         for (int r = 0; r < P; ++r) buf[r * NT + tid] = x[r];
         __syncthreads();
@@ -153,12 +154,12 @@
       }
     }
   }
-  __syncthreads();
+  if constexpr (WAVE) wave_lds_sync(); else __syncthreads();
   if (tid * P < n_out) {
 #pragma unroll
     for (int r = 0; r < P; ++r) buf[tid * P + r] = x[r];
   }
-  __syncthreads();
+  if constexpr (WAVE) wave_lds_sync(); else __syncthreads();
 }
 
 template <int NT, int CAP = 0>
```

New measurement: 3.236 million query spectra/s (median of 6 runs). +2.3%, better.
